# leggedrobotics/open3d_slam_private

Measured on AMD Instinct MI355X. Metric: ICP iterations/sec (scan-to-map), higher is better.
Workload: dtype f32

## Files before the change

### include/o3dslam_reg_debug.h

```cpp
#ifndef O3DSLAM_REG_DEBUG_H
#define O3DSLAM_REG_DEBUG_H

#include "o3dslam_reg.h"

#ifdef __cplusplus
extern "C" {
#endif

typedef struct {
    int32_t struct_size;
    int32_t profile_loop;
    int32_t match_variant;
    int32_t debug_flags;
    int32_t disable_halo;
    int32_t lanes_per_point;
    int32_t disable_fused;
    int32_t reserved;
} reg_debug_params;

REG_API reg_status reg_debug_configure(reg_handle* h, const reg_debug_params* d);

REG_API reg_status reg_debug_halo_bound(reg_handle* h, const float* xyz, int64_t n, float* out);

REG_API reg_status reg_debug_halo_witness(reg_handle* h, const float* xyz, int64_t n, int32_t* out);

REG_API reg_status reg_debug_live_resources(int64_t out[4]);

#ifdef __cplusplus
}
#endif
#endif
```

### open3d_slam_private_amd/capi.py

```python
from __future__ import annotations

import ctypes as C
import math
import os
import subprocess
import weakref

import numpy as np

_HERE = os.path.dirname(os.path.abspath(__file__))
_SO = os.environ.get("O3D_REG_LIB") or os.path.join(_HERE, "lib", "libo3dslam_reg.so")

STATUS_NAMES = {0: "OK", 1: "EMPTY_TARGET", 2: "EMPTY_SOURCE", 3: "NO_CORRESPONDENCES", 4: "BAD_TRANSFORM",
                5: "NOT_CONFIGURED", 6: "BAD_ARGUMENT", 7: "MISSING_FIELD", 8: "DEVICE_ERROR", 9: "UNSUPPORTED",
                10: "OUT_OF_BOUNDS"}
OUT_OF_BOUNDS = 10
COST_P2PL, COST_GICP = 0, 1
COST_O3D_P2PL, COST_O3D_P2P = 2, 3
SMOOTH_LEN_MAX = 15


class RegError(RuntimeError):
    def __init__(self, status, msg=""):
        self.status = status
# ... 276 lines not shown
def host_scan_key(seed: int, index: int) -> int:
    return int(load_library().reg_host_scan_key(int(seed), int(index)))


def default_scan_params(**overrides) -> ScanParams:
    p = ScanParams()
    load_library().reg_default_scan_params(C.byref(p))
    for k, v in overrides.items():
        if k in ("wide", "narrow"):
            v = Registration._crop_struct(v if v is not None else {"type": CROP_NONE})
        elif not hasattr(p, k):
            raise TypeError(f"unknown scan parameter {k}")
        setattr(p, k, v)
    p.struct_size = C.sizeof(ScanParams)
    return p


def host_ransac_est_k(est_k, confidence, count, k, ransac_n) -> float:
    return float(load_library().reg_host_ransac_est_k(float(est_k), float(confidence), int(count), int(k), int(ransac_n)))


class OctreeOut(C.Structure):
    _fields_ = [("xyz", C.c_void_p), ("normals", C.c_void_p), ("covs", C.c_void_p), ("src_idx", C.c_void_p),
                ("leaf_id", C.c_void_p), ("leaf_depth", C.c_void_p)]


class PmChain(C.Structure):
    _fields_ = [("struct_size", C.c_int32), ("knn", C.c_int32), ("minimizer", C.c_int32), ("use_robust", C.c_int32),
                ("robust_fct", C.c_int32), ("tuning", C.c_float), ("scale_estimator", C.c_int32),
                ("nb_iter_for_scale", C.c_int32), ("distance_type", C.c_int32), ("approximation", C.c_float),
                ("reserved", C.c_int32 * 2),
                ("use_min_dist_filter", C.c_int32), ("outlier_min_dist", C.c_float),
                ("use_median_dist", C.c_int32), ("median_factor", C.c_float),
                ("use_var_trimmed", C.c_int32), ("var_min_ratio", C.c_float), ("var_max_ratio", C.c_float),
                ("var_lambda", C.c_float)]


class PmChainV3(PmChain):
    _fields_ = [("with_cov", C.c_int32), ("sensor_std_dev", C.c_float),
                ("use_bound", C.c_int32), ("max_rotation_norm", C.c_float), ("max_translation_norm", C.c_float),
                ("bound_after_counter", C.c_int32),
                ("degeneracy_method", C.c_int32), ("sr_threshold", C.c_float), ("sr_use2019", C.c_int32),
                ("reserved2", C.c_int32)]


class MinimizerStats(C.Structure):
    _fields_ = [("struct_size", C.c_int32), ("returned_prior", C.c_int32), ("point_used_ratio", C.c_double),
                ("weighted_point_used_ratio", C.c_double), ("overlap", C.c_double), ("residual_error", C.c_double),
                ("n_rejected_matches", C.c_int64), ("n_rejected_points", C.c_int64)]


class TernaryXicp(C.Structure):
    _fields_ = [("struct_size", C.c_int32), ("enabled", C.c_int32), ("high_information", C.c_float),
                ("enough_information", C.c_float), ("insufficient_information", C.c_float),
                ("min_alignment_angle_deg", C.c_float), ("strong_alignment_angle_deg", C.c_float), ("reserved", C.c_int32)]


class TernaryXicpResult(C.Structure):
    _fields_ = [("struct_size", C.c_int32), ("iteration", C.c_int32), ("category", C.c_int32 * 6), ("sane", C.c_int32),
                ("reserved", C.c_int32), ("combined", C.c_double * 6), ("high", C.c_double * 6),
                ("n_combined", C.c_int64 * 6), ("n_high", C.c_int64 * 6), ("n_pairs", C.c_int64),
                ("constraint", C.c_float * 6), ("partial_sums", (C.c_double * 9) * 6), ("eigenvectors", (C.c_float * 9) * 2)]


TERNARY_LOCALIZABLE, TERNARY_PARTIAL_MIXED, TERNARY_PARTIAL_HIGH, TERNARY_NONE = 0, 1, 2, 3
PM_CHAIN_SIZE_V1 = 48
PM_CHAIN_SIZE_V2 = 80
DEGENERACY_NONE, DEGENERACY_SOLUTION_REMAPPING = 0, 1
PM_POINT_TO_PLANE, PM_POINT_TO_POINT = 0, 1
ROBUST_FCTS = {"cauchy": 0, "welsch": 1, "sc": 2, "gm": 3, "tukey": 4, "huber": 5, "L1": 6, "student": 7}
SCALE_ESTIMATORS = {"none": 0, "mad": 1, "berg": 2, "std": 3}
DISTANCE_TYPES = {"point2point": 0, "point2plane": 1}


EXPORTS = ["reg_default_params", "reg_shipped_params", "reg_create", "reg_destroy", "reg_last_error",
           "reg_set_stream", "reg_set_target", "reg_set_source", "reg_register", "reg_compute", "reg_prepare",
           "reg_linearize", "reg_get_correspondences", "reg_match_local", "reg_trim_histogram", "reg_reduce_local",
           "reg_solve_update", "reg_host_solve6", "reg_host_x_to_T", "reg_host_centroid", "reg_get_target_info", "reg_profile_kernels", "reg_source_centroid_sums", "reg_prepare_centroid", "reg_compose",
           "reg_dist_begin", "reg_dist_buffers", "reg_dist_phase", "reg_dist_finish",
           "reg_dist_fused_buffers", "reg_dist_poll", "reg_estimate_normals", "reg_smooth_normals", "reg_host_solve6_xicp",
           "reg_set_target_f64", "reg_get_target_source_indices", "reg_voxelize_within_volume", "reg_carve_indices", "reg_dist_xicp_buffers", "reg_dist_gather_buffers",
           "reg_dist_record", "reg_dist_centroid_sums", "reg_dist_prepare",
           "reg_information_matrix", "reg_set_source_f64", "reg_debug_configure", "reg_debug_halo_bound", "reg_debug_halo_witness",
           "reg_debug_live_resources",
           "reg_dist_get_unique_id", "reg_dist_init", "reg_dist_init_custom", "reg_dist_register", "reg_dist_shutdown",
           "reg_dist_info", "reg_dist_steer_create", "reg_dist_steer_destroy", "reg_dist_steer_step",
           "reg_dist_steer_counts", "reg_host_tail_plan", "reg_host_o3d_update",
           "reg_default_pm_chain", "reg_check_pm_chain", "reg_set_pm_chain", "reg_get_robust_state",
           "reg_get_correspondences_k", "reg_host_robust_weights", "reg_host_pm_p2p_update",
           "reg_get_var_trim", "reg_host_var_trim",
           "reg_get_covariance", "reg_get_covariance_sums", "reg_host_censi_covariance", "reg_get_minimizer_stats",
           "reg_get_degeneracy", "reg_get_bound", "reg_host_solution_remap",
           "reg_default_ternary_xicp", "reg_check_ternary_xicp", "reg_set_ternary_xicp", "reg_get_ternary_xicp",
           "reg_host_ternary_decide", "reg_host_partial_constraint", "reg_host_solve6_xicp_rhs",
           "reg_default_ssn_params", "reg_sampling_surface_normal", "reg_filter_points",
           "reg_default_octree_params", "reg_octree_grid", "reg_host_octree_root", "reg_host_octree_random_picks",
           "reg_filter_cloud", "reg_host_glibc_rand", "reg_default_voxel_grid_params", "reg_voxel_grid",
           "reg_overlap_indices", "reg_set_pair_overlap_f64", "reg_get_source_source_indices",
           "reg_compute_fpfh", "reg_match_features", "reg_ransac_correspondences", "reg_host_ransac_est_k",
           "reg_voxel_down_sample", "reg_random_down_sample", "reg_host_scan_key", "reg_default_scan_params",
           "reg_process_scan",
           "reg_dense_map_create", "reg_dense_map_destroy", "reg_dense_map_clear", "reg_dense_map_insert",
           "reg_default_dense_scan_params", "reg_dense_map_insert_scan", "reg_default_dense_carve_params",
           "reg_dense_map_carve", "reg_dense_map_transform", "reg_dense_map_center", "reg_dense_map_get_info",
           "reg_dense_map_export", "reg_dedup_voxels", "reg_host_dense_offsets"]


def lib_path() -> str:
    return _SO


def build_library(force: bool = False) -> str:
    src_dir = os.path.join(_HERE, "csrc")
    cmd = ["make", "-C", src_dir]
    if force:
        cmd.append("-B")
    subprocess.check_call(cmd)
    return _SO


_lib = None


def load_library():
    global _lib
    if _lib is not None:
        return _lib
    if not os.path.exists(_SO):
        raise ImportError(f"{_SO} is missing: build it with `python -c 'import __graft_entry__ as g; g.build()'` "
                          "(hipcc --offload-arch=gfx950).  There is no CPU fallback for the registration path.")
    lib = C.CDLL(_SO)
    vp, i64, f32p = C.c_void_p, C.c_int64, C.c_void_p
    lib.reg_create.argtypes = [C.POINTER(RegParams), C.POINTER(vp)]
    lib.reg_destroy.argtypes = [vp]
    lib.reg_last_error.argtypes = [vp]
    lib.reg_last_error.restype = C.c_char_p
    lib.reg_set_stream.argtypes = [vp, vp]
    lib.reg_debug_configure.argtypes = [vp, C.POINTER(RegDebugParams)]
    lib.reg_debug_halo_bound.argtypes = [vp, f32p, i64, f32p]
    lib.reg_debug_halo_witness.argtypes = [vp, f32p, i64, vp]
    lib.reg_debug_live_resources.argtypes = [C.POINTER(C.c_int64)]
    lib.reg_dist_get_unique_id.argtypes = [C.c_char_p]
    lib.reg_dist_init.argtypes = [vp, C.c_char_p, C.c_int, C.c_int]
    lib.reg_dist_init_custom.argtypes = [vp, C.POINTER(Collectives), C.c_int, C.c_int]
    lib.reg_dist_register.argtypes = [vp, f32p, f32p, C.POINTER(RegResult)]
    lib.reg_dist_shutdown.argtypes = [vp]
    lib.reg_dist_info.argtypes = [vp, C.POINTER(C.c_int64), C.POINTER(C.c_int32), C.POINTER(C.c_int32), C.POINTER(C.c_int32)]
    lib.reg_dist_steer_create.argtypes = [C.c_int, C.c_int, C.c_int, C.c_float, C.c_int]
    lib.reg_dist_steer_create.restype = vp
    lib.reg_dist_steer_destroy.argtypes = [vp]
    lib.reg_dist_steer_destroy.restype = None
    lib.reg_dist_steer_step.argtypes = [vp, C.POINTER(DistReply)]
    lib.reg_dist_steer_step.restype = DistAction
    lib.reg_dist_steer_counts.argtypes = [vp, C.POINTER(C.c_int32), C.POINTER(C.c_int32), C.POINTER(C.c_int32)]
    lib.reg_dist_steer_counts.restype = None
    lib.reg_set_source_f64.argtypes = [vp, vp, vp, vp, i64, C.c_int]
    lib.reg_set_target.argtypes = [vp, f32p, i64, f32p, i64, f32p, i64, C.c_int]
    lib.reg_set_source.argtypes = [vp, f32p, i64, f32p, i64, f32p, i64, C.c_int]
    lib.reg_register.argtypes = [vp, f32p, f32p, C.POINTER(RegResult)]
    lib.reg_compute.argtypes = [vp, f32p, i64, f32p, i64, f32p, i64, C.c_int, f32p, f32p, C.POINTER(RegResult)]
    lib.reg_prepare.argtypes = [vp, f32p]
    lib.reg_linearize.argtypes = [vp, f32p, f32p, f32p, C.POINTER(C.c_double), C.POINTER(C.c_int64)]
    lib.reg_get_correspondences.argtypes = [vp, vp, vp, vp]
    lib.reg_match_local.argtypes = [vp, f32p]
    lib.reg_trim_histogram.argtypes = [vp, C.c_int, C.c_uint32, vp]
    lib.reg_reduce_local.argtypes = [vp, f32p, C.c_float, vp]
    lib.reg_solve_update.argtypes = [C.POINTER(RegParams), vp, f32p, f32p, C.POINTER(C.c_int32)]
    lib.reg_host_solve6.argtypes = [f32p, f32p, f32p]
    lib.reg_host_solve6.restype = C.c_int
    lib.reg_host_x_to_T.argtypes = [f32p, f32p]
    lib.reg_host_solve6_xicp.argtypes = [f32p, f32p, vp, f32p]
    lib.reg_host_solve6_xicp.restype = C.c_int
    lib.reg_set_target_f64.argtypes = [vp, vp, vp, vp, i64, C.c_int, C.POINTER(RegCrop), C.POINTER(C.c_int64)]
    lib.reg_get_target_source_indices.argtypes = [vp, vp]
    lib.reg_carve_indices.argtypes = [vp, vp, vp, i64, vp, i64, C.c_int, C.POINTER(C.c_double), C.POINTER(RegCrop),
                                      C.c_double, C.c_double, C.c_double, C.c_double, vp, C.POINTER(C.c_int64)]
    lib.reg_voxelize_within_volume.argtypes = [vp, vp, vp, vp, i64, C.c_int, C.POINTER(RegCrop), C.c_double, vp, vp, vp,
                                               C.POINTER(C.c_int64), C.POINTER(C.c_int64)]
    lib.reg_overlap_indices.argtypes = [vp, vp, i64, vp, i64, C.c_int, C.POINTER(C.c_double), C.c_double, C.c_int32, vp,
                                        C.POINTER(C.c_int64), vp, C.POINTER(C.c_int64)]
    lib.reg_set_pair_overlap_f64.argtypes = [vp, vp, vp, vp, i64, vp, vp, vp, i64, C.c_int, C.POINTER(C.c_double), C.c_double,
                                             C.c_int32, C.POINTER(C.c_int64), C.POINTER(C.c_int64)]
    lib.reg_get_source_source_indices.argtypes = [vp, vp]
    lib.reg_compute_fpfh.argtypes = [vp, vp, i64, vp, i64, i64, C.c_int, C.c_int, C.c_float, vp, vp, vp, C.POINTER(C.c_int64)]
    lib.reg_match_features.argtypes = [vp, vp, i64, vp, i64, C.c_int, C.c_int, vp, vp, vp, C.POINTER(C.c_int64)]
    lib.reg_ransac_correspondences.argtypes = [vp, vp, i64, vp, i64, vp, i64, C.c_int, C.POINTER(RansacParams),
                                               C.POINTER(RansacResult), vp, vp]
    lib.reg_host_ransac_est_k.argtypes = [C.c_double, C.c_double, i64, i64, C.c_int32]
    lib.reg_host_ransac_est_k.restype = C.c_double
    lib.reg_voxel_down_sample.argtypes = [vp, vp, vp, vp, i64, C.c_int, C.c_double, vp, vp, vp, C.POINTER(C.c_int64)]
    lib.reg_random_down_sample.argtypes = [vp, vp, vp, vp, i64, C.c_int, C.c_double, C.c_uint64, vp, vp, vp, vp,
                                           C.POINTER(C.c_int64)]
    lib.reg_host_scan_key.argtypes = [C.c_uint64, C.c_uint64]
    lib.reg_host_scan_key.restype = C.c_uint64
    lib.reg_default_scan_params.argtypes = [C.POINTER(ScanParams)]
    lib.reg_default_scan_params.restype = None
    lib.reg_process_scan.argtypes = [vp, vp, vp, vp, i64, C.c_int, C.POINTER(ScanParams), vp, vp, vp, C.POINTER(ScanResult)]
    pd16, pi64 = C.POINTER(C.c_double), C.POINTER(C.c_int64)
    lib.reg_dense_map_create.argtypes = [vp, C.c_double, C.POINTER(vp)]
    lib.reg_dense_map_destroy.argtypes = [vp]
    lib.reg_dense_map_destroy.restype = None
    lib.reg_dense_map_clear.argtypes = [vp]
    lib.reg_dense_map_insert.argtypes = [vp, vp, vp, vp, i64, C.c_int, pd16, pi64, pi64]
    lib.reg_default_dense_scan_params.argtypes = [C.POINTER(DenseScanParams)]
    lib.reg_default_dense_scan_params.restype = None
    lib.reg_dense_map_insert_scan.argtypes = [vp, vp, vp, vp, i64, C.c_int, C.POINTER(DenseScanParams), pd16, pi64, pi64]
    lib.reg_default_dense_carve_params.argtypes = [C.POINTER(DenseCarveParams)]
    lib.reg_default_dense_carve_params.restype = None
    lib.reg_dense_map_carve.argtypes = [vp, vp, i64, C.c_int, pd16, C.POINTER(DenseCarveParams), vp, pi64]
    lib.reg_dense_map_transform.argtypes = [vp, pd16]
    lib.reg_dense_map_center.argtypes = [vp, pd16]
    lib.reg_dense_map_get_info.argtypes = [vp, C.POINTER(DenseMapInfo)]
    lib.reg_dense_map_export.argtypes = [vp, C.c_int, vp, vp, vp, vp, vp, i64, pi64]
    lib.reg_dedup_voxels.argtypes = [vp, vp, i64, C.c_int, C.c_double, vp, pi64]
    lib.reg_host_dense_offsets.argtypes = [C.c_double, C.c_double, vp]
    lib.reg_host_dense_offsets.restype = C.c_int32
    lib.reg_host_centroid.argtypes = [f32p, i64, i64, f32p]
    lib.reg_host_o3d_update.argtypes = [C.c_int, vp, vp, C.POINTER(C.c_int32)]
    lib.reg_get_target_info.argtypes = [vp, C.POINTER(TargetInfo)]
    lib.reg_profile_kernels.argtypes = [vp, f32p, C.c_int, f32p]
    lib.reg_source_centroid_sums.argtypes = [vp, vp]
    lib.reg_prepare_centroid.argtypes = [vp, f32p, f32p]
    lib.reg_compose.argtypes = [vp, f32p, f32p]
    lib.reg_dist_begin.argtypes = [vp, f32p]
# ... 872 lines not shown
            out["normals"] = np.zeros((n, 3), np.float32)
        if cv is not None:
            out["covs"] = np.zeros((n, 6), np.float32)
        o = OctreeOut()
        for key in ("xyz", "normals", "covs", "src_idx", "leaf_id", "leaf_depth"):
            setattr(o, key, out[key].ctypes.data if key in out else None)
        m = C.c_int64(0)
        self._check(self._lib.reg_octree_grid(self._h, _ptr(xyz), xyz.shape[1] if xyz.ndim == 2 else 3, _ptr(nr), _ptr(cv),
                                              n, 0, C.byref(p), C.byref(o), C.byref(m)))
        for key in ("xyz", "src_idx", "normals", "covs"):
            if key in out:
                out[key] = out[key][:m.value].copy()
        out["n_out"] = int(m.value)
        return out

    def octree_grid_device(self, xyz_ptr, xyz_stride, n, params: "OctreeParams", xyz_out_ptr, nrm_ptr=None, cov_ptr=None,
                           normals_out_ptr=None, covs_out_ptr=None, src_idx_ptr=None, leaf_id_ptr=None,
                           leaf_depth_ptr=None) -> int:
        o = OctreeOut(xyz_out_ptr, normals_out_ptr, covs_out_ptr, src_idx_ptr, leaf_id_ptr, leaf_depth_ptr)
        m = C.c_int64(0)
        self._check(self._lib.reg_octree_grid(self._h, C.c_void_p(xyz_ptr), xyz_stride, nrm_ptr, cov_ptr, n, 1,
                                              C.byref(params), C.byref(o), C.byref(m)))
        return int(m.value)

    def smooth_normals(self, normals, ids):
        nr = np.ascontiguousarray(normals, dtype=np.float32).copy()
        ii = np.ascontiguousarray(ids, dtype=np.int32)
        passes = C.c_int32(0)
        self._check(self._lib.reg_smooth_normals(self._h, _ptr(nr), _ptr(ii), nr.shape[0], ii.shape[1], 0, C.byref(passes)))
        return nr, int(passes.value)

    def estimate_normals_device(self, xyz_ptr, xyz_stride, n, normals_ptr, k=10, max_dist=np.inf, viewpoint=None,
                                regularise=False, eigvals_ptr=None, covs_ptr=None, ids_ptr=None, eigvecs_ptr=None,
                                densities_ptr=None, mean_dists_ptr=None):
        vp_ = _f32(viewpoint) if viewpoint is not None else None
        o = NormalsOut()
        o.normals, o.eigvals, o.eigvecs, o.covs = normals_ptr, eigvals_ptr, eigvecs_ptr, covs_ptr
        o.densities, o.mean_dists, o.ids = densities_ptr, mean_dists_ptr, ids_ptr
        resc = C.c_int64(0)
        self._check(self._lib.reg_estimate_normals(
            self._h, C.c_void_p(xyz_ptr), xyz_stride, n, 1, int(k), float(max_dist), _ptr(vp_), 1 if regularise else 0,
            C.byref(o), C.byref(resc)))
        return int(resc.value)

    def set_target_device(self, xyz_ptr, xyz_stride, m, nrm_ptr=None, nrm_stride=3, cov_ptr=None):
        self._check(self._lib.reg_set_target(self._h, C.c_void_p(xyz_ptr), xyz_stride,
                                             C.c_void_p(nrm_ptr) if nrm_ptr else None, nrm_stride,
                                             C.c_void_p(cov_ptr) if cov_ptr else None, m, 1))

    def set_source_device(self, xyz_ptr, xyz_stride, n, nrm_ptr=None, nrm_stride=3, cov_ptr=None):
        self._check(self._lib.reg_set_source(self._h, C.c_void_p(xyz_ptr), xyz_stride,
                                             C.c_void_p(nrm_ptr) if nrm_ptr else None, nrm_stride,
                                             C.c_void_p(cov_ptr) if cov_ptr else None, n, 1))
        self.n_source = n

    def register(self, T_init=None):
        Ti = _T_in(np.eye(4) if T_init is None else T_init)
        To = np.zeros(16, np.float32)
        res = RegResult()
        st = self._lib.reg_register(self._h, _ptr(Ti), _ptr(To), C.byref(res))
        self.last_result = res
        self._check(st)
        return _T_out(To), res

    def information_matrix(self, T, max_dist):
        Ti = _T_in(T)
        info = (C.c_double * 36)()
        n = C.c_int64(0)
        self._check(self._lib.reg_information_matrix(self._h, _ptr(Ti), float(max_dist), info, C.byref(n)))
        return np.array(info[:], np.float64).reshape(6, 6), int(n.value)

    def halo_bound(self, xyz):
        x = _f32(xyz)
        out = np.empty(x.shape[0], np.float32)
        self._check(self._lib.reg_debug_halo_bound(self._h, _ptr(x), x.shape[0], _ptr(out)))
        return out

    def halo_witness(self, xyz):
        x = _f32(xyz)
        out = np.empty(x.shape[0], np.int32)
        self._check(self._lib.reg_debug_halo_witness(self._h, _ptr(x), x.shape[0], _ptr(out)))
        return out

    def prepare(self, T_init=None):
        Ti = _T_in(np.eye(4) if T_init is None else T_init)
        self._check(self._lib.reg_prepare(self._h, _ptr(Ti)))

    def linearize(self, T_iter=None):
        Ti = _T_in(np.eye(4) if T_iter is None else T_iter)
        H = np.zeros(36, np.float32)
        b = np.zeros(6, np.float32)
        err = C.c_double()
        cnt = C.c_int64()
        self._check(self._lib.reg_linearize(self._h, _ptr(Ti), _ptr(H), _ptr(b), C.byref(err), C.byref(cnt)))
        return H.reshape(6, 6), b, err.value, cnt.value

    def correspondences(self, want_w=True):
        n = self.n_source
        ids = np.empty(n, np.int32)
        d2 = np.empty(n, np.float32)
        w = np.empty(n, np.float32) if want_w else None
        self._check(self._lib.reg_get_correspondences(self._h, _ptr(ids), _ptr(d2), _ptr(w)))
        return ids, d2, w

    def set_pm_chain(self, chain: "PmChain | None"):
        if chain is not None:
            chain.struct_size = C.sizeof(type(chain))
        self.pm_chain = chain
        self._check(self._lib.reg_set_pm_chain(self._h, C.byref(chain) if chain is not None else None))

    def set_ternary_xicp(self, ternary: "TernaryXicp | None"):
        if ternary is not None:
            ternary.struct_size = C.sizeof(TernaryXicp)
        self._check(self._lib.reg_set_ternary_xicp(self._h, C.byref(ternary) if ternary is not None else None))
        self.ternary_xicp = ternary

    def get_ternary_xicp(self) -> TernaryXicpResult:
        out = TernaryXicpResult()
        out.struct_size = C.sizeof(TernaryXicpResult)
        self._check(self._lib.reg_get_ternary_xicp(self._h, C.byref(out)))
        return out

    def get_correspondences_k(self, knn=None, want_w=True):
        if knn is None:
            knn = self.pm_chain.knn if getattr(self, "pm_chain", None) is not None else 1
        n = self.n_source
        ids = np.empty((n, knn), np.int32)
        d2 = np.empty((n, knn), np.float32)
        w = np.empty((n, knn), np.float32) if want_w else None
        self._check(self._lib.reg_get_correspondences_k(self._h, int(knn), _ptr(ids), _ptr(d2), _ptr(w)))
        return ids, d2, w

    def robust_state(self):
        sc = C.c_float()
        it = C.c_int32()
        self._check(self._lib.reg_get_robust_state(self._h, C.byref(sc), C.byref(it)))
        return float(sc.value), int(it.value)

    def get_var_trim(self):
        ratio, k, n = C.c_float(), C.c_int64(), C.c_int64()
        self._check(self._lib.reg_get_var_trim(self._h, C.byref(ratio), C.byref(k), C.byref(n)))
        return float(ratio.value), int(k.value), int(n.value)

    def get_covariance(self):
        cov = np.zeros(36, np.float32)
        rank = C.c_int32()
        self._check(self._lib.reg_get_covariance(self._h, _ptr(cov), C.byref(rank)))
        return cov.reshape(6, 6), int(rank.value)

    def get_covariance_sums(self):
        Hp, Mp = np.zeros(21, np.float64), np.zeros(21, np.float64)
        self._check(self._lib.reg_get_covariance_sums(self._h, _ptr(Hp), _ptr(Mp)))
        return unpack_sym6(Hp), unpack_sym6(Mp)

    def get_minimizer_stats(self) -> MinimizerStats:
        st = MinimizerStats()
        st.struct_size = C.sizeof(MinimizerStats)
        self._check(self._lib.reg_get_minimizer_stats(self._h, C.byref(st)))
        return st

    def get_degeneracy(self):
        cat, eig, cond = np.zeros(6, np.int32), np.zeros(6, np.float32), C.c_float()
        self._check(self._lib.reg_get_degeneracy(self._h, _ptr(cat), _ptr(eig), C.byref(cond)))
        return cat, eig, float(cond.value)

    def get_bound(self):
# ... 253 lines not shown
        return self._lib.reg_dist_steer_step(self._s, C.byref(reply) if reply is not None else None)

    def counts(self):
        g, f, s = C.c_int32(), C.c_int32(), C.c_int32()
        self._lib.reg_dist_steer_counts(self._s, C.byref(g), C.byref(f), C.byref(s))
        return g.value, f.value, s.value

    def __del__(self):
        try:
            if self._s:
                self._lib.reg_dist_steer_destroy(self._s)
                self._s = None
        except Exception:
            pass


def solve_update(params: RegParams, sums, T_iter):
    lib = load_library()
    s = np.ascontiguousarray(sums, np.float64)
    To = np.zeros(16, np.float32)
    rank = C.c_int32()
    st = lib.reg_solve_update(C.byref(params), _ptr(s), _ptr(_T_in(T_iter)), _ptr(To), C.byref(rank))
    if st != 0:
        raise RegError(st, "reg_solve_update")
    return _T_out(To), rank.value


def host_solve6(A, b):
    x = np.zeros(6, np.float32)
    rank = load_library().reg_host_solve6(_ptr(_f32(A).reshape(36)), _ptr(_f32(b)), _ptr(x))
    return x, rank


def host_solve6_xicp(A, b, flags):
    x = np.zeros(6, np.float32)
    f = np.ascontiguousarray(flags, np.int32)
    rank = load_library().reg_host_solve6_xicp(_ptr(_f32(A).reshape(36)), _ptr(_f32(b)), _ptr(f), _ptr(x))
    return x, rank


def host_x_to_T(x):
    T = np.zeros(16, np.float32)
    load_library().reg_host_x_to_T(_ptr(_f32(x)), _ptr(T))
    return _T_out(T)


def host_centroid(xyz):
    xyz = _f32(xyz)
    out = np.zeros(3, np.float32)
    load_library().reg_host_centroid(_ptr(xyz), xyz.shape[1], xyz.shape[0], _ptr(out))
    return out


def host_o3d_update(cost, sums):
    s = np.ascontiguousarray(sums, np.float64).reshape(32)
    U = np.zeros(16, np.float64)
    rank = C.c_int32()
    st = load_library().reg_host_o3d_update(int(cost), _ptr(s), _ptr(U), C.byref(rank))
    if st != 0:
        raise RegError(st, "reg_host_o3d_update")
    return U.reshape(4, 4).T.copy(), rank.value


def host_tail_plan(n, cus=256, tile=0):
    lib = load_library()
    lib.reg_host_tail_plan.argtypes = [C.c_int64, C.c_int32, C.c_int32, C.POINTER(C.c_int32)]
    lib.reg_host_tail_plan.restype = None
    out = (C.c_int32 * 4)()
    lib.reg_host_tail_plan(int(n), int(cus), int(tile), out)
    return bool(out[0]), int(out[1]), int(out[2]), int(out[3])


def host_predict_band(limit, prev=math.inf, prev2=math.inf, last_count=0, last_lo=math.inf, last_hi=math.inf, debug_narrow=0):
    lib = load_library()
    lib.reg_host_predict_band.argtypes = [C.c_float, C.c_float, C.c_float, C.c_uint32, C.c_float, C.c_float, C.c_int32,
                                          C.POINTER(C.c_float), C.POINTER(C.c_float)]
    lib.reg_host_predict_band.restype = None
    out = (C.c_float * 2)()
    lib.reg_host_predict_band(float(limit), float(prev), float(prev2), int(last_count), float(last_lo), float(last_hi),
                              int(debug_narrow), out, None)
    return np.float32(out[0]), np.float32(out[1])


def host_band_constants():
    lib = load_library()
    lib.reg_host_predict_band.argtypes = [C.c_float, C.c_float, C.c_float, C.c_uint32, C.c_float, C.c_float, C.c_int32,
                                          C.POINTER(C.c_float), C.POINTER(C.c_float)]
    lib.reg_host_predict_band.restype = None
    c = (C.c_float * 8)()
    lib.reg_host_predict_band(math.inf, math.inf, math.inf, 0, math.inf, math.inf, 0, None, c)
    names = ("band_cap", "wide_rel", "floor", "ratio_max", "centre_gain", "geom_rel", "guard_frac", "forced_wide")
    return {k: float(np.float32(v)) for k, v in zip(names, c)}
```

### open3d_slam_private_amd/csrc/host_handle.hpp

```cpp
#pragma once

struct EnvSwitches {
    bool trace = false;
    bool event_timing = false;
    bool halo_occ = true;
    bool no_dynprune = false;
    bool no_empty_bound = false;
    bool no_witness = false;
    bool no_burst = false;
    bool hints = false;
    bool stamps = false;
    bool coh_stats = false;
    bool tail_always = false;
    bool update_generic = false;
    bool no_tail = false;
    int tail_wpc = 0;
    double dist_timeout_s = 30.0;
    float tail_timeout_s = 2.f;
    int xcd_tile_first = 32;
    int xcd_tile_later = 16;
    float settle_trans = 0.02f;
    float settle_rot = 4e-3f;
    int tail_min_iters = 8;
    int tail_tile = 0;
    bool no_gicp_tail = false;
    int gicp_tail_after = 1;
    float tail_settle_tol = 1.2f;
    int lookahead = 2;
    float settle_tol = 0.05f;
    float halo_ratio = 1.25f;
    float halo_rho = 0.4f;
    float reach_bins = 7.25f;
    float bin_occupancy = 8.f;
    float level_ratio = 2.0f;
    void read() {
        trace = getenv("O3D_TRACE") != nullptr;
        event_timing = getenv("O3D_EVENT_TIMING") != nullptr;
        no_burst = getenv("O3D_NO_BURST") != nullptr;
        no_dynprune = getenv("O3D_NO_DYNPRUNE") != nullptr;
        no_empty_bound = getenv("O3D_NO_EMPTY_BOUND") != nullptr;
        no_witness = getenv("O3D_NO_WITNESS") != nullptr;
        halo_occ = getenv("O3D_NO_HALO_OCC") == nullptr;
        hints = getenv("O3D_HINTS") != nullptr;
        stamps = getenv("O3D_STAMPS") != nullptr;
        coh_stats = getenv("O3D_COH_STATS") != nullptr;
        tail_always = getenv("O3D_TAIL_ALWAYS") != nullptr;
        no_tail = getenv("O3D_NO_TAIL") != nullptr;
        if (const char* v = getenv("O3D_UPDATE_GENERIC")) update_generic = atoi(v) != 0;
        if (const char* v = getenv("O3D_TAIL_WPC")) tail_wpc = std::max(0, atoi(v));
        if (const char* v = getenv("O3D_DIST_TIMEOUT_S")) dist_timeout_s = std::max(0.5, atof(v));
        if (const char* v = getenv("O3D_TAIL_SETTLE")) tail_settle_tol = (float)atof(v);
        if (const char* v = getenv("O3D_NO_GICP_TAIL")) no_gicp_tail = atoi(v) != 0;
        if (const char* v = getenv("O3D_TAIL_TILE")) tail_tile = std::max(0, atoi(v));
        if (const char* v = getenv("O3D_TAIL_MIN_ITERS")) tail_min_iters = std::max(0, atoi(v));
        if (const char* v = getenv("O3D_SETTLE_TRANS")) settle_trans = (float)atof(v);
        if (const char* v = getenv("O3D_SETTLE_ROT")) settle_rot = (float)atof(v);
        if (const char* v = getenv("O3D_XCD_TILE_FIRST")) xcd_tile_first = std::max(0, atoi(v));
        if (const char* v = getenv("O3D_XCD_TILE_LATER")) xcd_tile_later = std::max(0, atoi(v));
        if (const char* v = getenv("O3D_GICP_TAIL_AFTER")) gicp_tail_after = atoi(v);
        if (const char* v = getenv("O3D_TAIL_TIMEOUT_S")) tail_timeout_s = std::min(30.f, std::max(0.01f, (float)atof(v)));
        if (const char* v = getenv("O3D_KAHEAD")) lookahead = std::max(1, atoi(v));
        if (const char* v = getenv("O3D_SETTLE")) settle_tol = (float)atof(v);
        if (const char* v = getenv("O3D_HALO_RATIO")) halo_ratio = std::min(4.0f, std::max(0.5f, (float)atof(v)));
        if (const char* v = getenv("O3D_HALO_RHO")) halo_rho = std::min(1.0f, std::max(0.05f, (float)atof(v)));
        if (const char* v = getenv("O3D_REACH_BINS")) reach_bins = std::max(1.0f, (float)atof(v));
        if (const char* v = getenv("O3D_BIN_OCC")) bin_occupancy = std::min(64.0f, std::max(1.0f, (float)atof(v)));
        if (const char* v = getenv("O3D_LEVEL_RATIO")) level_ratio = std::min(4.0f, std::max(1.2f, (float)atof(v)));
    }
};

struct DistCtx;

struct reg_handle {
    reg_params prm;
    reg_debug_params dbg;
    EnvSwitches env;
    std::string err;
    Stream stream;
    Event ev0, ev1, ev_iter, ev_s0, ev_s1;
    Event ev_p0, ev_p1;
    std::vector<Event> prof_ev;
    Pinned<HostMirror> h_mirror;
    Pinned<IterState> h_iter;
    Pinned<PrepState> h_prep;
    bool device_ok = false;
    bool structure_only = false;
    reg_handle* normals_ws = nullptr;
    DevBuf n_out, n_ids, n_extra, n_mom;
    DevBuf fp_xyz, fp_nrm, fp_ids, fp_cnt, fp_out, fp_misc, mf_a, mf_b, mf_part, mf_nn, mf_flags;
    DevBuf rs_src, rs_tgt, rs_cor, rs_pairs, rs_batch, rs_part, rs_rec;
    std::vector<RsRecord> rs_head;
    DevBuf i_xicp;
    DevBuf c_in_xyz, c_in_nrm, c_in_cov, c_flags, c_offs, c_xyz, c_nrm, c_cov, c_idx;
    DevBuf r_in_xyz, r_in_nrm, r_in_cov, r_xyz, r_nrm, r_cov;
    int64_t crop_kept = 0;
    DevBuf v_fout, v_oout, v_out;
    DevBuf v_ukeys, v_ustart;
    DevBuf ov_keys[2], ov_sorted, ov_ukeys[2], ov_ucnt[2], ov_flags[2], ov_offs[2], ov_misc, ov_sidx;
    DevBuf i_info;
    int64_t src_kept = 0;
    DevBuf sp_in[3], sp_a[3], sp_b[3], sp_c[3], sp_f32[3], sp_keys, sp_keys2, sp_vals, sp_vals2, sp_flags, sp_offs, sp_part,
        sp_misc;
    DevBuf dm_in[3], dm_crop[3], dm_tf[2], dm_keys, dm_keys2, dm_vals, dm_vals2, dm_heads, dm_run, dm_rank, dm_new, dm_newoff,
        dm_newkeys, dm_mark, dm_keep, dm_off1, dm_off2, dm_misc, dm_out;
    DevBuf d_d2all;
    int64_t dist_nmax = 0;
    int dist_gather_ranks = 0;
    bool xicp_pending = false;
    bool src_prep_pending = false;
    float source_prep_ms = 0.f;
    int rotation_corrected = 0;
    bool iter_copy_pending = false;

    int64_t m = 0;
    bool has_tnrm = false, has_tcov = false;
    float c_ref[3] = {0, 0, 0};
    float t_mid[3] = {0, 0, 0};
    DevBuf t_raw, t_nrm_raw, t_cov_raw, t_centred, t_keys, t_keys2, t_vals, t_vals2, t_pts, t_nrm, t_cov, t_flags,
        t_scan, t_hash, t_cells, t_misc, t_dir, t_rows;
    DevBuf rp_tmp;
    Grid grid;
    reg_target_info info;
    float target_build_ms = 0.f;

    int64_t n = 0;
    bool has_snrm = false, has_scov = false, prepared = false;
    int64_t s_stride = 3, s_nstride = 3;
    float c_read[3] = {0, 0, 0};
    DevBuf s_raw, s_nrm_raw, s_cov_raw, s_xyz, s_nrm, s_cov, s_misc;
    float T_init[16];
    float T0[16];
    DevBuf i_pos, i_d2, i_w, i_hist, i_state, i_partials, i_sums, i_ids;
    DevBuf i_iter;
    unsigned long long seq = 0;
    DevBuf t_halo_start, t_halo_cursor, t_halo_pts, t_halo_dir, i_band, i_acc, i_cache, i_stats, i_queue, i_qcount;
    DevBuf s_prep;
    int cent_slot = 0;
    bool prep_pending = false;
    DevBuf i_hint, s_keys, s_keys2, s_perm, s_perm2, s_tmp, i_tmpf;
    const uint32_t* perm = nullptr;
    int last_stalls = 0;
    int64_t n_total_hint = 0;
    int match_launches = 0;
    int tail_sync_slot = 0, tail_sync_last = 0;
    bool tail_sync_dirty = true;
    int last_tail_launches = 0, last_tail_iters = 0;
    DevBuf i_tail_sync, i_tail_rows, i_tail_band;
    unsigned long long dist_seq0 = 0;
    DevBuf d_contrib, d_gathered;
    int dist_ranks = 0, dist_rank = 0;
    DistCtx* dist = nullptr;
    unsigned long long src_epoch = 0;
    std::vector<int> prof_kind;
    bool profiling = false;
    int shift0 = 21;
    int n_blocks = 0;
    bool have_match = false;
    bool pm_on = false;
    reg_pm_chain pm;
    bool pm_have_match = false;
    DevBuf pm_pos, pm_d2, pm_w, pm_keys, pm_hist, pm_sel, pm_state, pm_partials;
    DevBuf pm_sorted, pm_sort_tmp, pm_var;
    size_t pm_sort_bytes = 0;
    DevBuf pm_xstate, pm_xrows, pm_xmeans, pm_xcov;
    PmExtraState pm_xhost;
    PmCovOut pm_cov_host;
    bool pm_x_valid = false;
    bool pm_cov_valid = false;
    float pm_cov_ms = 0.f;
    double pm_last_error = 0.0;
    bool xt_on = false;
    reg_ternary_xicp xt;
    DevBuf xt_state, xt_rows;
    XtState xt_host;
    bool xt_valid = false;
    DevBuf f_in, f_in_nrm, f_in_cov, f_px, f_pn, f_pc, f_perm, f_keys, f_keys2, f_segs, f_boxes, f_boxes2, f_leaf,
        f_mom, f_mom2, f_lid, f_keep, f_pos, f_misc, f_out;
    DevBuf f_fields, f_draws;
    DevBuf o_keys, o_keys_s, o_iota, o_idx, o_idx2, o_rank, o_rank_a, o_rank_s, o_c, o_kk, o_heads, o_pos, o_open, o_depth,
        o_start, o_rand, o_radii;
};
static_assert(!std::is_copy_constructible<DevBuf>::value && !std::is_copy_constructible<reg_handle>::value, "owners are not copied");

#define HIPCHK(h, call)                                                                        \
    do {                                                                                       \
        hipError_t e_ = (call);                                                                \
        if (e_ != hipSuccess) {                                                                \
            (h)->err = std::string(#call) + ": " + hipGetErrorString(e_);                      \
            return REG_DEVICE_ERROR;                                                           \
        }                                                                                      \
    } while (0)

static inline void col_to_row(const float* c, float* r) { m4_transpose(c, r); }
static inline void row_to_col(const float* r, float* c) { m4_transpose(r, c); }

static inline int grid_for(int64_t n, int block = 256) { return (int)((n + block - 1) / block); }

static inline bool cost_is_o3d(int cost) { return cost == REG_COST_O3D_P2PL || cost == REG_COST_O3D_P2P; }

static inline bool pm_needs_tnrm(const reg_handle* h) {
    return h->pm.minimizer == REG_PM_POINT_TO_PLANE || h->prm.use_surface_normal ||
           (h->pm.use_robust && h->pm.distance_type == REG_DIST_POINT2PLANE);
}

static reg_status check_target_fields(reg_handle* h, bool has_nrm, bool has_cov) {
    if ((h->prm.cost == REG_COST_P2PL || h->prm.cost == REG_COST_O3D_P2PL) && !has_nrm && !h->structure_only &&
        !(h->pm_on && !pm_needs_tnrm(h))) {
        h->err = "InvalidField: point-to-plane needs the `normals` descriptor on the reference";
        return REG_MISSING_FIELD;
    }
    if (h->prm.cost == REG_COST_GICP && !has_cov && !h->structure_only) {
        h->err = "InvalidField: GICP needs covariances on the reference";
        return REG_MISSING_FIELD;
    }
    return REG_OK;
}
static reg_status check_source_fields(reg_handle* h, bool has_nrm, bool has_cov) {
    if (h->prm.cost == REG_COST_P2PL && h->prm.use_surface_normal && !has_nrm) {
        h->err = "InvalidField: SurfaceNormalOutlierFilter needs the `normals` descriptor on the reading";
        return REG_MISSING_FIELD;
    }
    if (h->prm.cost == REG_COST_GICP && !has_cov) {
        h->err = "InvalidField: GICP needs covariances on the reading";
        return REG_MISSING_FIELD;
    }
    return REG_OK;
}

extern "C" {
// ... 203 lines not shown
```

### open3d_slam_private_amd/csrc/host_loop.hpp

```cpp
#pragma once


static reg_status check_ready(reg_handle* h, bool need_prepared) {
    if (!h) return REG_BAD_ARGUMENT;
    if (!h->device_ok) return REG_DEVICE_ERROR;
    if (h->m == 0) {
        h->err = "no reference set (reg_set_target)";
        return REG_NOT_CONFIGURED;
    }
    if (h->n == 0) {
        h->err = "no reading set (reg_set_source)";
        return REG_NOT_CONFIGURED;
    }
    if (need_prepared && !h->prepared) {
        h->err = "reg_prepare has not been called for this reading";
        return REG_NOT_CONFIGURED;
    }
    return REG_OK;
}

static reg_status prepare_rowmajor(reg_handle* h, const float* T_init_row, const float* c_override = nullptr,
                                   int64_t n_global = 0, const IterState* init_state = nullptr) {
    reg_status s = check_ready(h, false);
    if (s != REG_OK) return s;
// ... 63 lines not shown
}


static void xicp_frame_change(const reg_handle* h, float Trd12[12]) {
    float A[16], Trd[16];
    m4_identity(A);
    for (int k = 0; k < 3; ++k) A[4 * k + 3] = -h->c_ref[k];
    m4_mul(A, h->T_init, Trd);
    for (int k = 0; k < 12; ++k) Trd12[k] = Trd[k];
}

static reg_status build_iter_state(reg_handle* h, const float* T_row, int update, IterState* st) {
    std::memset(st, 0, sizeof(IterState));
    for (int i = 0; i < 16; ++i) {
        st->T[i] = T_row[i];
        st->Td[i] = (double)T_row[i];
    }
    st->chk = Checkers();
    st->chk.max_iter = h->prm.max_iter;
    st->chk.min_diff_rot = h->prm.min_diff_rot;
    st->chk.min_diff_trans = h->prm.min_diff_trans;
    st->chk.smooth_len = h->prm.smooth_len;
    st->chk.init(T_row);
    st->cost = h->prm.cost;
    st->fixed_iters = h->prm.fixed_iters;
    st->max_iter = h->prm.max_iter;
    st->update = update;
    st->gicp_rot_eps = h->prm.gicp_rot_eps;
    st->gicp_trans_eps = h->prm.gicp_trans_eps;
    st->gicp_stop_rule = h->prm.gicp_stop_rule;
    st->gicp_rel_fitness = h->prm.gicp_rel_fitness;
    st->gicp_rel_rmse = h->prm.gicp_rel_rmse;
    st->n_total = (float)(h->n_total_hint > 0 ? h->n_total_hint : h->n);
    st->band_lo = st->band_hi = INFINITY;
    st->limit_last = st->limit_prev = st->limit_prev2 = INFINITY;
    st->use_trim = (h->prm.cost == REG_COST_P2PL && h->prm.use_trimmed) ? 1 : 0;
    st->trim_ratio = h->prm.trim_ratio;
    st->band_cap = kBandCap;
    st->qcount = h->i_qcount.as<unsigned int>();
    st->debug_narrow_band = ((h->dbg.debug_flags & 8) ? 1 : 0) | ((h->dbg.debug_flags & 64) ? 2 : 0);
    h->xicp_pending = false;
    for (int k = 0; k < 6; ++k) st->xicp_flags[k] = 1;
    if (h->prm.use_xicp && h->prm.cost == REG_COST_P2PL && update) {
        HIPCHK(h, h->i_xicp.reserve(sizeof(XicpState)));
        st->xicp_stage = 1;
        st->xicp_enough = h->prm.xicp_enough;
        st->xicp_insufficient = h->prm.xicp_insufficient;
        st->xicp_cos_min = (float)std::cos((double)h->prm.xicp_min_angle_deg * 3.14159265358979323846 / 180.0);
        st->xicp_cos_strong = (float)std::cos((double)h->prm.xicp_strong_angle_deg * 3.14159265358979323846 / 180.0);
        xicp_frame_change(h, st->xicp_Trd);
        h->xicp_pending = true;
    }
    return REG_OK;
}

static reg_status init_iter_state(reg_handle* h, const float* T_row, int update) {
    IterState* st = h->h_iter;
    if (h->iter_copy_pending) HIPCHK(h, hipEventSynchronize(h->ev_iter));
    reg_status s = build_iter_state(h, T_row, update, st);
    if (s != REG_OK) return s;
    HIPCHK(h, hipMemcpyAsync(h->i_iter.p, st, sizeof(IterState), hipMemcpyHostToDevice, h->stream));
    HIPCHK(h, hipEventRecord(h->ev_iter, h->stream));
    h->iter_copy_pending = true;
    return REG_OK;
}

static reg_status enqueue_match(reg_handle* h, bool zero_hist = false) {
    const bool trim = h->prm.cost == REG_COST_P2PL && h->prm.use_trimmed;
    if (trim && zero_hist) HIPCHK(h, hipMemsetAsync(h->i_hist.p, 0, 3 * 2048 * 4, h->stream));
    const bool fused_hist = h->dbg.match_variant == 3;
    uint32_t* hist0 = (trim && fused_hist) ? h->i_hist.as<uint32_t>() : nullptr;
    uint32_t* hist2 = trim ? h->i_hist.as<uint32_t>() + 4096 : nullptr;
    const IterState* it = h->i_iter.as<IterState>();
    if (h->dbg.match_variant == 1) {
        prof_mark(h, 0, true);
        k_match<<<h->n_blocks, 256, 0, h->stream>>>(h->s_xyz.as<float4>(), h->n, it, h->grid, h->i_pos.as<int>(),
                                                    h->i_d2.as<float>(), hist0, hist2, h->shift0);
        prof_mark(h, 0, false);
    } else {
        uint8_t* hint = h->dbg.match_variant == 2 ? nullptr : h->i_hint.as<uint8_t>();
        const int lanes = h->dbg.lanes_per_point == 4 ? 4 : (h->dbg.lanes_per_point == 2 ? 2 : 8);
        const int blocks = grid_for(h->n * lanes);
        const int tile = h->match_launches < 2 ? h->env.xcd_tile_first : h->env.xcd_tile_later;
        ++h->match_launches;
        const dim3 grid(xcd_tiled_grid(blocks, tile)), block(256);
        auto go = [&](auto kernel) {
            launch_timed(h, 0, kernel, grid, block, 0, (const float4*)h->s_xyz.as<float4>(), h->n, it, h->grid,
                         h->i_pos.as<int>(), h->i_d2.as<float>(), hist0, hist2, hint, h->shift0, h->dbg.debug_flags, blocks,
                         h->i_cache.as<float4>(), tile);
        };
        if (lanes == 4)
            go(k_match_g8<4>);
        else if (lanes == 2)
            go(k_match_g8<2>);
        else
            go(k_match_g8<8>);
    }
    h->have_match = true;
    return REG_OK;
}

static void enqueue_select(reg_handle* h) {
    const float* d2 = h->i_d2.as<float>();
    uint32_t* hist = h->i_hist.as<uint32_t>();
    SelectState* st = h->i_state.as<SelectState>();
    const int hb = std::min(h->n_blocks, 128);
    if (h->dbg.match_variant != 3) launch_hist_level0(h, d2, h->n, hb, hist);
    launch_select_level(h, 1, d2, h->n, hb, hist, st, h->prm.trim_ratio);
    launch_select_level(h, 2, d2, h->n, hb, hist, st, h->prm.trim_ratio);
}

static reg_status enqueue_linearize(reg_handle* h, bool want_w, bool limit_from_state = false) {
    float* w = want_w ? h->i_w.as<float>() : nullptr;
    if (h->prm.cost == REG_COST_P2PL) {
        launch_linearize_p2pl(h, h->prm.use_trimmed ? (limit_from_state ? 1 : 2) : 0, w);
    } else if (cost_is_o3d(h->prm.cost)) {
        const IterState* it = h->i_iter.as<IterState>();
        const float3 o = make_float3(h->t_mid[0], h->t_mid[1], h->t_mid[2]);
        if (h->prm.cost == REG_COST_O3D_P2PL)
            k_linearize_o3d<REG_COST_O3D_P2PL><<<h->n_blocks, 256, 0, h->stream>>>(
                h->s_xyz.as<float4>(), h->n, it, h->i_pos.as<int>(), h->i_d2.as<float>(), h->t_nrm.as<float4>(), o, w,
                h->i_partials.as<double>());
        else
            k_linearize_o3d<REG_COST_O3D_P2P><<<h->n_blocks, 256, 0, h->stream>>>(
                h->s_xyz.as<float4>(), h->n, it, h->i_pos.as<int>(), h->i_d2.as<float>(), h->t_pts.as<float4>(), o, w,
                h->i_partials.as<double>());
        update_o3d_from_partials(h);
        return REG_OK;
    } else {
        launch_linearize_gicp(h, w);
    }
    update_from_partials(h);
    if (h->xicp_pending) {
        h->xicp_pending = false;
        launch_xicp_center(h, h->i_pos.as<int>(), h->i_w.as<float>());
        launch_xicp_detect(h, h->i_pos.as<int>(), h->i_w.as<float>());
        update_xicp_finish(h);
    }
    return REG_OK;
}

static reg_status enqueue_fused(reg_handle* h) {
    CohStats* stats = h->env.coh_stats ? h->i_stats.as<CohStats>() : nullptr;
    const int rows = h->dbg.lanes_per_point == 4 ? launch_fused_search<4>(h, h->i_band.as<float>(), (int)kBandCap, stats, true)
                                                 : launch_fused_search<8>(h, h->i_band.as<float>(), (int)kBandCap, stats, true);
    update_fused_from_band(h, rows);
    h->have_match = true;
    return REG_OK;
}

constexpr int kTailMaxDevices = 64;
static std::mutex g_tail_mutex[kTailMaxDevices];
static std::atomic<int> g_reg_active[kTailMaxDevices];
struct RegActiveGuard {
    int dev;
    explicit RegActiveGuard(int d) : dev(d >= 0 && d < kTailMaxDevices ? d : -1) {
        if (dev >= 0) g_reg_active[dev].fetch_add(1, std::memory_order_relaxed);
    }
    ~RegActiveGuard() {
        if (dev >= 0) g_reg_active[dev].fetch_sub(1, std::memory_order_relaxed);
    }
    bool alone() const { return dev >= 0 && g_reg_active[dev].load(std::memory_order_relaxed) == 1; }
};
static int g_tail_cus[kTailMaxDevices];
static std::mutex g_tail_probe_mutex;

struct TailPlan {
    bool ok = false;
    int grid = 0, wpc = 0, chunk8 = 0, tile = 0;
};

static int tail_device_cus(int dev) {
    if (dev < 0 || dev >= kTailMaxDevices) return -1;
    std::lock_guard<std::mutex> lk(g_tail_probe_mutex);
    if (g_tail_cus[dev] != 0) return g_tail_cus[dev];
    int cus = 0, nb = 0;
    hipError_t e = hipDeviceGetAttribute(&cus, hipDeviceAttributeMultiprocessorCount, dev);
    int nb2 = 0;
    if (e == hipSuccess)
        e = hipFuncSetAttribute(reinterpret_cast<const void*>(k_tail<false>), hipFuncAttributeMaxDynamicSharedMemorySize, kTailLdsBytes);
    if (e == hipSuccess)
        e = hipFuncSetAttribute(reinterpret_cast<const void*>(k_tail<true>), hipFuncAttributeMaxDynamicSharedMemorySize, kTailLdsBytes);
    if (e == hipSuccess)
        e = hipOccupancyMaxActiveBlocksPerMultiprocessor(&nb, reinterpret_cast<const void*>(k_tail<false>), kTailThreads, kTailLdsBytes);
    if (e == hipSuccess)
        e = hipOccupancyMaxActiveBlocksPerMultiprocessor(&nb2, reinterpret_cast<const void*>(k_tail<true>), kTailThreads, kTailLdsBytes);
    g_tail_cus[dev] = (e == hipSuccess && nb >= kTailWgsPerCu && nb2 >= kTailWgsPerCu && cus >= 8) ? cus : -1;
    (void)hipGetLastError();
    return g_tail_cus[dev];
}

static TailPlan tail_plan_for(int64_t n, int cus, int wpc_cap, int tile) {
    TailPlan pl;
    if (cus < 8 || n <= 0) return pl;
    int wpc_max = cus * kTailWgsPerCu / 8;
    if (wpc_cap > 0) wpc_max = std::min(wpc_max, wpc_cap);
    pl.wpc = (int)std::max<int64_t>(1, std::min<int64_t>(wpc_max, (n + 2047) / 2048));
    pl.tile = std::max(0, tile);
    const int64_t unit = 8 * (int64_t)std::max(1, pl.tile);
    pl.chunk8 = (int)((((n + 7) / 8) + unit - 1) / unit * unit);
    const int64_t octets = pl.chunk8 / 8, per_wg = (octets + pl.wpc - 1) / pl.wpc * 8;
    pl.grid = 8 * pl.wpc;
    pl.ok = per_wg <= kTailSlots;
    return pl;
}
static TailPlan tail_plan(const reg_handle* h) {
    if (cost_is_o3d(h->prm.cost)) return TailPlan();
    if (h->prm.cost == REG_COST_GICP && h->env.no_gicp_tail) return TailPlan();
    if (h->dbg.disable_fused == 1 || (h->dbg.debug_flags & (16 | 64 | 128)) || h->dbg.lanes_per_point == 4 || h->env.no_tail)
        return TailPlan();
    return tail_plan_for(h->n, tail_device_cus(h->prm.device), h->env.tail_wpc, h->env.tail_tile);
}

static void last_step_motion(const HostMirror* m, float* trans, float* rot) {
    const float* A = m->T;
    const float* B = m->T_prev;
    float R[9];
    for (int i = 0; i < 3; ++i)
        for (int j = 0; j < 3; ++j) R[3 * i + j] = A[4 * i + 0] * B[4 * j + 0] + A[4 * i + 1] * B[4 * j + 1] + A[4 * i + 2] * B[4 * j + 2];
    float t[3];
    for (int i = 0; i < 3; ++i) t[i] = A[4 * i + 3] - (R[3 * i + 0] * B[3] + R[3 * i + 1] * B[7] + R[3 * i + 2] * B[11]);
    *trans = std::sqrt(t[0] * t[0] + t[1] * t[1] + t[2] * t[2]);
    const float sx = 0.5f * (R[7] - R[5]), sy = 0.5f * (R[2] - R[6]), sz = 0.5f * (R[3] - R[1]);
    *rot = std::sqrt(sx * sx + sy * sy + sz * sz);
}

static reg_status enqueue_tail(reg_handle* h, const TailPlan& pl, int max_iters) {
    if (!h->i_tail_sync.p) h->tail_sync_dirty = true;
    HIPCHK(h, h->i_tail_sync.reserve(2 * (size_t)kTailSyncBytes));
    if (h->tail_sync_dirty) {
        HIPCHK(h, hipMemsetAsync(h->i_tail_sync.p, 0, 2 * (size_t)kTailSyncBytes, h->stream));
        h->tail_sync_dirty = false;
    }
    const int sync_slot = h->tail_sync_slot;
    h->tail_sync_slot ^= 1;
    h->tail_sync_last = sync_slot;
    unsigned* const sync_cur = h->i_tail_sync.as<unsigned>() + (size_t)sync_slot * (kTailSyncBytes / 4);
    unsigned* const sync_next = h->i_tail_sync.as<unsigned>() + (size_t)(sync_slot ^ 1) * (kTailSyncBytes / 4);
    HIPCHK(h, h->i_tail_rows.reserve((size_t)2 * pl.grid * kTailHistRow * 8));
    HIPCHK(h, h->i_tail_band.reserve((size_t)2 * kTailBandCap * kTailRec * 4));
    const FilterCfg f = make_filter_cfg(h, 0);
    TailCfg cfg;
    cfg.n = h->n;
    cfg.chunk8 = pl.chunk8;
    cfg.wpc = pl.wpc;
    cfg.tile = pl.tile;
    cfg.max_iters = std::max(1, std::min(max_iters, kTailMaxIters));
    cfg.slack = coherent_slack(h);
    cfg.seq = ++h->seq;
    cfg.timeout_ticks = (unsigned long long)(h->env.tail_timeout_s * 1e8);
    uint8_t* hint = h->dbg.match_variant == 2 ? nullptr : h->i_hint.as<uint8_t>();
    const bool gicp = h->prm.cost == REG_COST_GICP;
    const float4* s_attr = gicp ? (const float4*)h->s_cov.as<float4>() : (const float4*)(h->has_snrm ? h->s_nrm.as<float4>() : nullptr);
    const float4* t_attr = gicp ? (const float4*)h->t_cov.as<float4>() : (const float4*)h->t_nrm.as<float4>();
    auto go = [&](auto kernel) {
        launch_timed(h, 3, kernel, dim3(pl.grid), dim3(kTailThreads), kTailLdsBytes, (const float4*)h->s_xyz.as<float4>(), s_attr,
                     h->i_iter.as<IterState>(), h->grid, t_attr, f, h->i_pos.as<int>(), h->i_d2.as<float>(), h->i_w.as<float>(), hint,
                     h->i_cache.as<float4>(), sync_cur, h->i_tail_rows.as<double>(), h->i_tail_band.as<float>(), h->h_mirror.dev, cfg,
                     sync_next);
    };
    if (gicp)
        go(k_tail<true>);
    else
        go(k_tail<false>);
    HIPCHK(h, hipGetLastError());
    h->have_match = true;
    return REG_OK;
}

static reg_status enqueue_iteration(reg_handle* h, bool want_w) {
    reg_status s = enqueue_match(h);
    if (s != REG_OK) return s;
    if (h->prm.cost == REG_COST_P2PL && h->prm.use_trimmed) enqueue_select(h);
    return enqueue_linearize(h, want_w);
}

static inline unsigned long long mirror_seq(const reg_handle* h) {
    return __atomic_load_n(&h->h_mirror->seq, __ATOMIC_ACQUIRE);
}

static reg_status wait_seq(reg_handle* h, unsigned long long seq) {
    for (unsigned spins = 0;; ++spins) {
        if (mirror_seq(h) >= seq) return REG_OK;
        __builtin_ia32_pause();
        if ((spins & 0x3fff) == 0x3fff) {
            hipError_t e = hipStreamQuery(h->stream);
            if (e == hipSuccess) return REG_OK;
            if (e != hipErrorNotReady) {
                h->err = std::string("device fault while waiting for the iteration: ") + hipGetErrorString(e);
                return REG_DEVICE_ERROR;
            }
        }
    }
}

static reg_status iterate_once(reg_handle* h, const float* T_row, bool want_w) {
    reg_status s = init_iter_state(h, T_row, 0);
    if (s != REG_OK) return s;
    s = enqueue_iteration(h, want_w);
    if (s != REG_OK) return s;
    s = wait_seq(h, h->seq);
    if (s != REG_OK) return s;
    HIPCHK(h, hipGetLastError());
    return REG_OK;
}

static void sums_to_system(const double* sums, int cost, float* H, float* b) {
    if (cost == REG_COST_O3D_P2P) {
        std::memset(H, 0, 36 * sizeof(float));
        std::memset(b, 0, 6 * sizeof(float));
        return;
    }
    const bool p2pl = cost == REG_COST_P2PL;
    int k = 0;
    for (int a = 0; a < 6; ++a)
        for (int c = a; c < 6; ++c) {
            const float v = (float)sums[k++];
            H[6 * a + c] = v;
            H[6 * c + a] = v;
        }
    for (int a = 0; a < 6; ++a) b[a] = p2pl ? -(float)sums[21 + a] : (float)sums[21 + a];
}

static void compose_rowmajor(reg_handle* h, const float* T_iter, float* Tout_row, bool later_kernel_reported = false) {
    if (h->prep_pending) {
        if (!later_kernel_reported) (void)hipStreamSynchronize(h->stream);
        std::memcpy(h->c_read, h->h_prep->c_read, 12);
        std::memcpy(h->T0, h->h_prep->T0, 64);
        h->prep_pending = false;
    }
    if (h->prm.cost == REG_COST_P2PL) {
// ... 68 lines not shown
    }
    void acknowledge() {
        acked = std::max(acked, m_seq);
        completed = any ? h->h_mirror->iterations : 0;
        inflight = (int)(h->seq - acked);
    }
    reg_status wait_next() {
        const reg_status s = wait_seq(h, acked + 1);
        if (s != REG_OK) return s;
        if (mirror_seq(h) <= acked) {
            if (hipStreamQuery(h->stream) == hipSuccess && mirror_seq(h) <= acked) acked = h->seq;
        }
        return REG_OK;
    }
};

struct SteerInput {
    bool any;
    float limit_last, limit_prev, step_trans, step_rot;
    int completed, inflight, generic_left, limit;
};
struct SteerPolicy {
    bool trimming, can_fuse, p2pl, no_burst;
    bool use_tail = false, tail_off = false;
    int tail_min_iters, fixed;
    float fused_settle_tol, tail_settle_tol, settle_trans, settle_rot;
    explicit SteerPolicy(const reg_handle* h) {
        p2pl = h->prm.cost == REG_COST_P2PL;
        can_fuse = p2pl && h->dbg.disable_fused != 1;
        trimming = p2pl && h->prm.use_trimmed && h->prm.trim_ratio != 1.0f;
        no_burst = h->env.no_burst;
        fixed = h->prm.fixed_iters;
        tail_min_iters = fixed > 0 ? 0 : h->env.tail_min_iters;
        fused_settle_tol = h->env.settle_tol;
        tail_settle_tol = h->env.tail_settle_tol;
        settle_trans = h->env.settle_trans;
        settle_rot = h->env.settle_rot;
    }
};
struct SteerChoice {
    enum Kind { kGeneric, kFused, kTail } kind;
    int count;
};

static SteerChoice steer_choose(const SteerInput& in, const SteerPolicy& p) {
    const bool tail_now = p.use_tail && !p.tail_off && in.completed + in.inflight >= p.tail_min_iters;
    const float settle_tol = tail_now ? p.tail_settle_tol : p.fused_settle_tol;
    bool settled = true;
    if (p.trimming) {
        settled = in.any && in.limit_prev < INFINITY && in.limit_last < INFINITY &&
                  std::fabs(in.limit_last - in.limit_prev) <= settle_tol * in.limit_last;
    }
    if (settled && in.any && (p.p2pl || p.fixed <= 0) && (p.can_fuse || tail_now)) {
        if (in.step_trans > p.settle_trans || in.step_rot > p.settle_rot) settled = false;
    }
    if (!(p.can_fuse || tail_now) || in.generic_left > 0 || !settled) return {SteerChoice::kGeneric, 1};
    const int rest = in.limit - (in.completed + in.inflight);
    if (tail_now) return {SteerChoice::kTail, rest};
    return {SteerChoice::kFused, p.fixed > 0 && !p.no_burst ? rest : 1};
}

static reg_status wait_tail(reg_handle* h, unsigned long long tail_seq, Lookahead& la, bool* tail_off) {
    const HostMirror* mir = h->h_mirror;
    for (unsigned spins = 0;; ++spins) {
        const unsigned long long m = mirror_seq(h);
        if (m >= tail_seq) break;
        if (m + 1 == tail_seq) {
            const HostMirror::SeqRecord* rec = &mir->ring[(tail_seq - 1) % kSeqRing];
            if (__atomic_load_n(&rec->seq, __ATOMIC_ACQUIRE) == tail_seq - 1 && (rec->done || rec->stall)) break;
        }
        __builtin_ia32_pause();
        if ((spins & 0xfff) == 0xfff) {
            const hipError_t e = hipStreamQuery(h->stream);
            if (e == hipSuccess) break;
            if (e != hipErrorNotReady) {
                h->tail_sync_dirty = true;
                h->err = std::string("device fault while waiting for the tail kernel: ") + hipGetErrorString(e);
                return REG_DEVICE_ERROR;
            }
        }
    }
    const bool reported = mirror_seq(h) >= tail_seq;
    const unsigned* sync_last = h->i_tail_sync.as<unsigned>() + (size_t)h->tail_sync_last * (kTailSyncBytes / 4);
    unsigned words[4] = {0, 0, 0, 0};
    if (!reported || h->env.coh_stats || mir->status == REG_DEVICE_ERROR)
        (void)hipMemcpy(words, sync_last + kTailErrWord, sizeof(words), hipMemcpyDeviceToHost);
    if (words[0] != 0 || (reported && mir->status == REG_DEVICE_ERROR)) {
        h->tail_sync_dirty = true;
        h->err = "persistent tail kernel: a grid barrier timed out (workgroups not co-resident? another process "
                 "running a persistent kernel on this GPU?); set O3D_NO_TAIL=1 to use the three-launch iteration";
        return REG_DEVICE_ERROR;
    }
    if (!reported && !(mir->stall && std::max(mirror_seq(h), la.seq0) > la.acked)) la.acked = h->seq;
    if (h->env.coh_stats)
        fprintf(stderr, "[o3dreg] tail launch: %u iterations, %u point searches (%.2f %% of the point-iterations), stall cause %u, band records of its last iteration %d\n", words[2],
                words[1], words[2] ? 100.0 * words[1] / ((double)words[2] * (double)h->n) : 0.0, words[3], reported ? mir->pad_nband : -1);
    if (reported) h->last_tail_iters += mir->pad3;
    if (reported && mir->stall && h->prm.fixed_iters <= 0) *tail_off = true;
#if O3D_TAIL_STAMPS
    {
        unsigned long long st[24];
        (void)hipMemcpy(st, sync_last + kTailStampWord, sizeof(st), hipMemcpyDeviceToHost);
        const double it_n = std::max(1, reported ? mir->pad3 : 1);
        static const char* names[12] = {"check", "search", "epilogue", "bandrec+comps", "sum+publish+drain", "arrive+wait", "row sums",
                                        "band-stage", "band-scan", "band-rank", "band-add", "solve+update"};
        for (int wg = 0; wg < 2; ++wg) {
            fprintf(stderr, "[o3dreg] tail stamps (us per iteration, %s workgroup):", wg ? "last" : "first");
            for (int i = 0; i < 12; ++i) fprintf(stderr, " %s %.2f", names[i], st[12 * wg + i] * 0.01 / it_n);
            fprintf(stderr, "\n");
        }
    }
#endif
    return REG_OK;
}

static reg_status loop_time_end(reg_handle* h, bool event_timing, std::chrono::steady_clock::time_point t_begin, float* loop_ms) {
    if (event_timing) {
        HIPCHK(h, hipEventRecord(h->ev1, h->stream));
        HIPCHK(h, hipEventSynchronize(h->ev1));
        (void)hipEventElapsedTime(loop_ms, h->ev0, h->ev1);
    } else {
        *loop_ms = std::chrono::duration<float, std::milli>(std::chrono::steady_clock::now() - t_begin).count();
    }
    return REG_OK;
}

static void loop_end_diagnostics(reg_handle* h, reg_result* res) {
    const HostMirror* mir = h->h_mirror;
    if (h->env.hints) {
        std::vector<uint8_t> hv((size_t)h->n);
        if (hipMemcpy(hv.data(), h->i_hint.p, (size_t)h->n, hipMemcpyDeviceToHost) == hipSuccess) {
            long long cnt[18] = {0};
            for (uint8_t v : hv) ++cnt[v < 17 ? v : 17];
            fprintf(stderr, "[o3dreg] terminating level of the last iteration (halo, then levels with rho =");
            for (int l = 0; l < h->grid.n_levels; ++l) fprintf(stderr, " %.3f", h->grid.rho[l]);
            fprintf(stderr, "):");
            for (int l = 0; l <= h->grid.n_levels; ++l) fprintf(stderr, " %lld", cnt[l]);
            fprintf(stderr, "\n");
        }
    }
    if (h->env.coh_stats) {
        CohStats cs;
        if (hipMemcpy(&cs, h->i_stats.p, sizeof(cs), hipMemcpyDeviceToHost) == hipSuccess) {
            fprintf(stderr, "[o3dreg] coherent fused iterations: %llu point-iterations, %llu searched (%.2f %%)\n", cs.n_points,
                    cs.n_searched, cs.n_points ? 100.0 * (double)cs.n_searched / (double)cs.n_points : 0.0);
            (void)hipMemset(h->i_stats.p, 0, sizeof(cs));
        }
    }
    if (h->env.stamps) {
        fprintf(stderr, "update kernel stamps (cycles): reduce %llu [rows %llu select %llu band-add %llu] solve %llu update+check %llu mirror %llu\n", mir->stamps[0],
                mir->stamps[4], mir->stamps[5], mir->stamps[6], mir->stamps[1], mir->stamps[2], mir->stamps[3]);
        fprintf(stderr, "   select detail: verify+stage-issue %llu, zero+hist+barriers %llu, wave0 pick/rank %llu\n", mir->stamps[3], mir->stamps[7] >> 32, mir->stamps[7] & 0xffffffffull);
    }
    if (h->profiling) {
        for (size_t i = 0; i + 1 < h->prof_ev.size(); i += 2) {
            float ms = 0;
            if (hipEventElapsedTime(&ms, h->prof_ev[i], h->prof_ev[i + 1]) == hipSuccess) {
                const int kind = h->prof_kind[i / 2];
                res->prof_ms[kind] += ms;
                res->prof_launches[kind] += 1;
            }
        }
        h->prof_ev.clear();
        h->prof_kind.clear();
        h->profiling = false;
    }
}

static reg_status register_pm(reg_handle* h, const float* Ti, float T_out[16], reg_result* res);

extern "C" {

void reg_host_tail_plan(int64_t n, int32_t cus, int32_t tile, int32_t plan[4]) {
    const TailPlan pl = tail_plan_for(n, cus, 0, tile);
    plan[0] = pl.ok ? 1 : 0;
    plan[1] = pl.grid;
    plan[2] = pl.wpc;
    plan[3] = pl.chunk8;
}

REG_API void reg_host_predict_band(float limit, float prev, float prev2, uint32_t last_count, float last_lo, float last_hi,
                                   int32_t debug_narrow, float band[2], float consts[8]) {
    const Band b = predict_band(limit, prev, prev2, last_count, last_lo, last_hi, debug_narrow);
    if (band) {
        band[0] = b.lo;
        band[1] = b.hi;
    }
    if (consts) {
        const float c[8] = {(float)kTailBandCap, kTailWideRel, kBandFloor, kBandRatioMax, kBandCentreGain, kBandGeomRel, kBandGuardFrac,
                            kBandForcedWide};
        for (int i = 0; i < 8; ++i) consts[i] = c[i];
    }
}

reg_status reg_prepare(reg_handle* h, const float T_init[16]) {
    if (!h || !T_init) return REG_BAD_ARGUMENT;
    float Tr[16];
    col_to_row(T_init, Tr);
    return prepare_rowmajor(h, Tr);
}

reg_status reg_linearize(reg_handle* h, const float T_iter[16], float H[36], float b[6], double* err,
                         int64_t* n_inliers) {
    reg_status s = check_ready(h, true);
    if (s != REG_OK) return s;
    if (!T_iter) return REG_BAD_ARGUMENT;
    if (h->prm.cost == REG_COST_O3D_P2P) {
        h->err = "reg_linearize: point-to-point (Umeyama) has no normal equations";
        return REG_UNSUPPORTED;
    }
    if (h->pm_on) {
        h->err = "reg_linearize: not available with a libpointmatcher chain (reg_set_pm_chain)";
        return REG_UNSUPPORTED;
    }
    float Tr[16];
    col_to_row(T_iter, Tr);
    if (!m4_is_finite(Tr)) return REG_BAD_TRANSFORM;
    HIPCHK(h, hipSetDevice(h->prm.device));
    s = iterate_once(h, Tr, true);
    if (s != REG_OK) return s;
    const double* sums = h->h_mirror->sums;
    if (H && b) sums_to_system(sums, h->prm.cost, H, b);
    if (err) *err = sums[27];
    if (n_inliers) *n_inliers = (int64_t)llround(sums[28]);
    if (sums[28] == 0.0) {
        h->err = "ErrorMinimizer: no point to minimize";
        return REG_NO_CORRESPONDENCES;
    }
    return REG_OK;
}

reg_status reg_register(reg_handle* h, const float T_init[16], float T_out[16], reg_result* res) {
    if (!h || !T_init || !T_out) return REG_BAD_ARGUMENT;
    reg_result local;
    if (!res) res = &local;
    std::memset(res, 0, sizeof(*res));
    std::memcpy(T_out, T_init, 64);
    float Ti[16];
    col_to_row(T_init, Ti);
    const auto t_reg0 = std::chrono::steady_clock::now();
    auto rmark = [&](const char* what) {
        if (h->env.trace)
            fprintf(stderr, "[o3dreg] register %-14s t=%.1fus\n", what,
                    std::chrono::duration<double, std::micro>(std::chrono::steady_clock::now() - t_reg0).count());
    };
    if (h->pm_on) return register_pm(h, Ti, T_out, res);
    const bool p2pl = h->prm.cost == REG_COST_P2PL;
    float T_start[16];
    if (p2pl)
        m4_identity(T_start);
    else
        std::memcpy(T_start, Ti, 64);
    std::memcpy(h->T_init, Ti, 64);
    IterState st0;
    reg_status s = build_iter_state(h, T_start, 1, &st0);
    if (s != REG_OK) return s;
    rmark("iter state");
    s = prepare_rowmajor(h, Ti, nullptr, 0, &st0);
    if (s != REG_OK) return s;
    rmark("prepared");
    h->profiling = h->dbg.profile_loop != 0;
    h->prof_ev.clear(), h->prof_kind.clear();
    const bool event_timing = h->profiling || h->env.event_timing;
    if (event_timing) HIPCHK(h, hipEventRecord(h->ev0, h->stream));
    const auto t_loop_begin = std::chrono::steady_clock::now();
    rmark("ev0");
    Lookahead la{h, h->seq, h->seq};
    SteerPolicy pol(h);
    const TailPlan tail_pl = (pol.can_fuse || h->prm.cost == REG_COST_GICP) ? tail_plan(h) : TailPlan();
    const RegActiveGuard active(h->prm.device);
    std::unique_lock<std::mutex> tail_lock;
    if (tail_pl.ok && (active.alone() || h->env.tail_always)) {
        tail_lock = std::unique_lock<std::mutex>(g_tail_mutex[h->prm.device], std::try_to_lock);
    }
    pol.use_tail = tail_pl.ok && tail_lock.owns_lock();
    const int limit = sequence_limit(h->prm);
    const int kAhead = h->env.lookahead;
    const HostMirror* mir = h->h_mirror;
    int generic_left = pol.trimming ? 2 : (h->prm.cost == REG_COST_GICP ? std::max(1, h->env.gicp_tail_after) : 1);
    unsigned long long last_traced = 0;
    const auto t_loop0 = std::chrono::steady_clock::now();
    unsigned long long tail_seq = 0;
    h->last_stalls = h->last_tail_launches = h->last_tail_iters = 0;
    for (;;) {
        if (tail_seq) {
            s = wait_tail(h, tail_seq, la, &pol.tail_off);
            if (s != REG_OK) return s;
            tail_seq = 0;
            continue;
        }
        la.look();
        if (la.any && mir->done) break;
        if (la.any && mir->stall && la.m_seq > la.acked) {
            HIPCHK(h, hipStreamSynchronize(h->stream));
            la.acked = h->seq;
            generic_left = 2;
            ++h->last_stalls;
            continue;
        }
        if (h->env.trace && la.m_seq != last_traced) {
            last_traced = la.m_seq;
            float mt = 0.f, mr = 0.f;
            last_step_motion(mir, &mt, &mr);
            fprintf(stderr, "[o3dreg] seq %llu iter %d stall %d band_n %d limit %.6g prev %.6g band [%.6g, %.6g) step %.2e m %.2e rad\n",
                    la.m_seq - la.seq0, mir->iterations, mir->stall, mir->stall ? mir->band_count : mir->pad_nband, mir->limit_last,
                    mir->limit_prev, mir->band_lo, mir->band_hi, mt, mr);
        }
        la.acknowledge();
        if (la.completed + la.inflight < limit && la.inflight < kAhead) {
            SteerInput seen = {la.any, mir->limit_last, mir->limit_prev, 0.f, 0.f, la.completed, la.inflight, generic_left, limit};
            if (la.any) last_step_motion(mir, &seen.step_trans, &seen.step_rot);
            const SteerChoice c = steer_choose(seen, pol);
            const auto tq0 = std::chrono::steady_clock::now();
            if (c.kind == SteerChoice::kGeneric) {
                s = enqueue_iteration(h, true);
                if (generic_left > 0) --generic_left;
            } else if (c.kind == SteerChoice::kTail) {
                s = enqueue_tail(h, tail_pl, c.count);
                tail_seq = h->seq;
                ++h->last_tail_launches;
            } else {
                for (int burst = c.count; burst > 0 && s == REG_OK; --burst) s = enqueue_fused(h);
            }
            if (h->env.trace) {
                const auto tq1 = std::chrono::steady_clock::now();
                fprintf(stderr, "[o3dreg] t=%.1fus enqueue seq %llu (%s) took %.1fus; mirror at %llu\n",
                        std::chrono::duration<double, std::micro>(tq0 - t_loop0).count(), h->seq - la.seq0,
                        c.kind == SteerChoice::kGeneric ? "generic" : (c.kind == SteerChoice::kTail ? "tail" : "fused"),
                        std::chrono::duration<double, std::micro>(tq1 - tq0).count(), std::max(mirror_seq(h), la.seq0) - la.seq0);
            }
            if (s != REG_OK) return s;
            continue;
        }
        if (la.inflight == 0) break;
        s = la.wait_next();
        if (s != REG_OK) return s;
    }
    rmark("loop done");
    s = loop_time_end(h, event_timing, t_loop_begin, &res->loop_ms);
    if (s != REG_OK) return s;
    HIPCHK(h, hipGetLastError());
    rmark("loop timed");
    loop_end_diagnostics(h, res);
    s = write_result(h, h->prm.use_xicp != 0, true, (double)h->n, true, T_out, res);
    if (s != REG_OK) {
        h->err = mir->sums[29] == 0.0 ? "No matches available for computing distance quantiles"
                                      : "ErrorMinimizer: no point to minimize";
        return s;
    }
    res->n_band_stalls = h->last_stalls;
    res->n_tail_launches = h->last_tail_launches;
    res->n_tail_iterations = h->last_tail_iters;
    rmark("return");
    return REG_OK;
}

reg_status reg_information_matrix(reg_handle* h, const float T[16], float max_dist, double info[36], int64_t* n_pairs) {
    if (!h || !T || !info) return REG_BAD_ARGUMENT;
    if (n_pairs) *n_pairs = 0;
    if (!(max_dist > 0.f) || max_dist > h->prm.max_dist) {
        h->err = "reg_information_matrix: max_dist must be positive and within the handle's max_dist";
        return REG_BAD_ARGUMENT;
    }
    float Tr[16];
    col_to_row(T, Tr);
    reg_status s = prepare_rowmajor(h, Tr);
    if (s != REG_OK) return s;
    float T_start[16];
    if (h->prm.cost == REG_COST_P2PL)
        m4_identity(T_start);
    else
        std::memcpy(T_start, Tr, 64);
    s = init_iter_state(h, T_start, 0);
    if (s != REG_OK) return s;
    s = enqueue_match(h, false);
    if (s != REG_OK) return s;
    h->have_match = true;
    const int blocks = (int)std::min<int64_t>(512, (h->n + 255) / 256);
    HIPCHK(h, h->i_info.reserve((size_t)512 * 10 * sizeof(double)));
    HIPCHK(h, hipMemsetAsync(h->i_info.p, 0, (size_t)blocks * 10 * sizeof(double), h->stream));
    k_info_sums<<<blocks, 256, 0, h->stream>>>(h->i_pos.as<int>(), h->i_d2.as<float>(), h->n, h->t_pts.as<float4>(),
                                               h->c_ref[0], h->c_ref[1], h->c_ref[2], max_dist * max_dist,
                                               h->i_info.as<double>());
    std::vector<double> rows((size_t)blocks * 10);
    HIPCHK(h, hipMemcpyAsync(rows.data(), h->i_info.p, rows.size() * sizeof(double), hipMemcpyDeviceToHost, h->stream));
    HIPCHK(h, hipStreamSynchronize(h->stream));
    HIPCHK(h, hipGetLastError());
    double m[10] = {0, 0, 0, 0, 0, 0, 0, 0, 0, 0};
    for (int b = 0; b < blocks; ++b)
        for (int k = 0; k < 10; ++k) m[k] += rows[(size_t)b * 10 + k];
    const double c = m[0], sx = m[1], sy = m[2], sz = m[3], xx = m[4], yy = m[5], zz = m[6], xy = m[7], xz = m[8], yz = m[9];
    const double I[36] = {yy + zz, -xy, -xz, 0, -sz, sy,
                          -xy, xx + zz, -yz, sz, 0, -sx,
                          -xz, -yz, xx + yy, -sy, sx, 0,
                          0, sz, -sy, c, 0, 0,
                          -sz, 0, sx, 0, c, 0,
                          sy, -sx, 0, 0, 0, c};
// ... 50 lines not shown
```

### open3d_slam_private_amd/csrc/kernels_fused.hpp

```cpp
#pragma once

constexpr int kBandCap = 16384;
constexpr int kContribHdr = 128;
__host__ __device__ __forceinline__ int contrib_cap_for(int n_ranks) {
    return n_ranks <= 1 ? 8192 : (n_ranks == 2 ? 4096 : (n_ranks <= 4 ? 2048 : (n_ranks <= 8 ? 1024 : 512)));
}
__host__ __device__ __forceinline__ size_t contrib_floats(int cap) { return (size_t)kContribHdr + (size_t)cap * 32; }
constexpr int kAccRows = 64;
constexpr int kRec = 32;
__host__ __device__ __forceinline__ size_t band_at(int comp, size_t slot) { return slot * kRec + (size_t)comp; }

__device__ __forceinline__ void p2pl_products(float3 p, float4 q, float4 nn, float w, float* vals) {
    float F[6];
    float a = p.y * nn.z, b = p.z * nn.y;
    F[0] = a - b;
    a = p.z * nn.x; b = p.x * nn.z;
    F[1] = a - b;
    a = p.x * nn.y; b = p.y * nn.x;
    F[2] = a - b;
    F[3] = nn.x; F[4] = nn.y; F[5] = nn.z;
    const float dx = p.x - q.x, dy = p.y - q.y, dz = p.z - q.z;
    float r = dx * nn.x;
    float t2 = dy * nn.y;
    r = r + t2;
// ... 237 lines not shown
            float bb = nr.y * nt.y;
            float val = a + bb;
            a = nr.z * nt.z;
            val = val + a;
            if (val < f.cos_max_angle) w = 0.f;
        }
        cls = md2 < band_lo ? 0 : (md2 < band_hi ? 1 : 2);
        row[9] = 1.f;
        if (cls == 0) row[11] = 1.f;
        if (w != 0.f && cls == 0) {
            float a = p.y * nn.z, bq = p.z * nn.y;
            row[0] = a - bq;
            a = p.z * nn.x; bq = p.x * nn.z;
            row[1] = a - bq;
            a = p.x * nn.y; bq = p.y * nn.x;
            row[2] = a - bq;
            row[3] = nn.x; row[4] = nn.y; row[5] = nn.z;
            const float dx = p.x - tq.x, dy = p.y - tq.y, dz = p.z - tq.z;
            float r = dx * nn.x;
            float t2 = dy * nn.y;
            r = r + t2;
            t2 = dz * nn.z;
            r = r + t2;
            row[6] = r;
            row[7] = 1.f;
            row[8] = 1.f;
            row[10] = md2;
        }
        if (cls == 1) write_band_record(it, band, band_cap, p, tq, nn, w, md2, (int)q);
    }
    pos_io[q] = mpos;
    d2_out[q] = mpos >= 0 ? md2 : INFINITY;
    if (w_out) w_out[q] = (cls == 2) ? 0.f : w;
}

__device__ __forceinline__ double coh_component(const float* E, int rows, int comp) {
    double acc = 0.0;
    if (comp < 28) {
        const int ia = kProdCode.a[comp] >> 2, ic = kProdCode.c[comp] >> 2;
        for (int i = 0; i < rows; ++i) {
            const float v = E[i * kCohRow + ia] * E[i * kCohRow + ic];
            acc += (double)v;
        }
    } else {
        const int ia = 8 + (comp - 28);
        for (int i = 0; i < rows; ++i) acc += (double)E[i * kCohRow + ia];
    }
    return acc;
}

__global__ void __launch_bounds__(256)
k_coh_check(const float4* __restrict__ src, const float4* __restrict__ src_nrm, int64_t n, IterState* __restrict__ it,
            Grid g, const float4* __restrict__ tgt_nrm, FilterCfg f, int* __restrict__ pos_io, float* __restrict__ d2_out,
            float* __restrict__ w_out, const float4* __restrict__ cache ,
            uint32_t* __restrict__ queue, int queue_cap, float* __restrict__ band, int band_cap, double* __restrict__ partials,
            int n_blocks) {
    __shared__ __attribute__((aligned(16))) float E[256 * kCohRow];
    __shared__ int s_wave_cnt[4];
    __shared__ unsigned s_base;
    __shared__ double sh[4][kSums];
    const int t = threadIdx.x;
    const int lb = xcd_block(n_blocks);
    const int64_t q = lb < n_blocks ? (int64_t)lb * 256 + t : n;
    const int64_t qc = q < n ? q : n - 1;
    const float4 s = src[qc];
    const float4 c = cache[qc];
    const float4 tq = cache[(size_t)n + qc];
    const float4 nn = cache[2 * (size_t)n + qc];
    const float4 ru = cache[3 * (size_t)n + qc];
    const int pprev = pos_io[qc];
    const int st_done = it->done, st_stall = it->stall;
    const Xf T = load_xf(it);
    const float band_lo = it->band_lo, band_hi = it->band_hi;
    unsigned int* const qcount = it->qcount;
#pragma unroll
    for (int k = 0; k < 12; ++k) asm volatile("" ::"s"(T.m[k]));
    asm volatile("" ::"s"(band_lo), "s"(band_hi));
    asm volatile("" ::"v"(s.x), "v"(c.w), "v"(pprev), "v"(tq.x), "v"(nn.x), "v"(ru.x));
    if ((st_done | st_stall) != 0) return;
    const float3 p = xf_point(T, s.x, s.y, s.z);
    bool pass = false;
    float md2 = INFINITY;
    if (q < n && c.w > 0.f && pprev >= 0 && nn.w == 1.f) {
        const float dx = p.x - tq.x, dy = p.y - tq.y, dz = p.z - tq.z;
        float a = dx * dx;
        float b = dy * dy;
        float d2 = a + b;
        a = dz * dz;
        d2 = d2 + a;
        const float ex = p.x - c.x, ey = p.y - c.y, ez = p.z - c.z;
        const float delta = __builtin_amdgcn_sqrtf(ex * ex + ey * ey + ez * ez);
        const float lhs = (__builtin_amdgcn_sqrtf(d2) + delta) * 1.00001f + 1e-30f;
        const float rhs = __builtin_amdgcn_sqrtf(c.w) * 0.99999f;
        pass = d2 <= g.max_d2 && lhs < rhs;
        if (ru.w == 1.f) {
            const float fx = p.x - ru.x, fy = p.y - ru.y, fz = p.z - ru.z;
            float a2 = fx * fx;
            float b2 = fy * fy;
            float r2 = a2 + b2;
            a2 = fz * fz;
            r2 = r2 + a2;
            pass = pass && d2 < r2;
        }
        md2 = d2;
    }
    const bool need = q < n && !pass;
    const unsigned long long bal = __ballot(need);
    const int lane = t & 63, wave = t >> 6;
    if (lane == 0) s_wave_cnt[wave] = (int)__popcll(bal);
    __syncthreads();
    if (t == 0) {
        const int tot = s_wave_cnt[0] + s_wave_cnt[1] + s_wave_cnt[2] + s_wave_cnt[3];
        s_base = tot ? atomicAdd(&qcount[(lb & (kQueues - 1)) * kQueueStride], (unsigned)tot) : 0u;
    }
    __syncthreads();
    if (need) {
        unsigned at = s_base + (unsigned)__popcll(bal & ((1ull << lane) - 1ull));
        for (int w2 = 0; w2 < wave; ++w2) at += (unsigned)s_wave_cnt[w2];
        queue[(size_t)(lb & (kQueues - 1)) * queue_cap + at] = (uint32_t)q;
    }
    float row[12];
    if (pass) {
        coh_epilogue(T, f, band_lo, band_hi, p, q, pprev, md2, tq, nn, src_nrm, it, band, band_cap, pos_io, d2_out, w_out, row);
    } else {
#pragma unroll
        for (int k = 0; k < 12; ++k) row[k] = 0.f;
    }
#pragma unroll
    for (int k = 0; k < 12; ++k) E[t * kCohRow + k] = row[k];
    __syncthreads();
    const int comp = t & (kSums - 1), part = t >> 5;
    double acc = coh_component(E + (part * 32) * kCohRow, 32, comp);
    acc += __shfl_xor(acc, 32);
    if (lane < kSums) sh[wave][lane] = acc;
    __syncthreads();
    if (t < kSums && lb < n_blocks) {
        const double tot = (sh[0][t] + sh[1][t]) + (sh[2][t] + sh[3][t]);
        unsafeAtomicAdd(&partials[(size_t)(lb & (kAccRows - 1)) * kSums + t], tot);
    }
}

template <int G>
__global__ void __launch_bounds__(256, O3D_SEARCH_WAVES)
k_coh_search(const float4* __restrict__ src, const float4* __restrict__ src_nrm, int64_t n, IterState* __restrict__ it,
             Grid g, const float4* __restrict__ tgt_nrm, FilterCfg f, int* __restrict__ pos_io, float* __restrict__ d2_out,
             float* __restrict__ w_out, uint8_t* __restrict__ hint, float4* __restrict__ cache,
             const uint32_t* __restrict__ queue, int queue_cap, float* __restrict__ band, int band_cap,
             double* __restrict__ partials, float slack, CohStats* __restrict__ stats) {
    constexpr int kQ = 256 / G;
    __shared__ __attribute__((aligned(16))) uint32_t seg_lds[kQ * kSegWords<G>];
    __shared__ __attribute__((aligned(16))) float E[kQ * kCohRow];
    __shared__ double sh[4][kSums];
    __shared__ unsigned s_pre[kQueues + 1];
    const int t = threadIdx.x;
    const int st_done = it->done, st_stall = it->stall;
    const Xf T = load_xf(it);
    const float band_lo = it->band_lo, band_hi = it->band_hi;
    const unsigned int* const qcount = it->qcount;
    if ((st_done | st_stall) != 0) return;
    if (t < 64) {
        static_assert(kQueues == 64, "one lane per sub-queue");
        const unsigned cnt = qcount[t * kQueueStride];
        unsigned incl = cnt;
#pragma unroll
        for (int o = 1; o < 64; o <<= 1) {
            const unsigned v = (unsigned)__shfl_up((int)incl, o);
            if (t >= o) incl += v;
        }
        s_pre[t + 1] = incl;
        if (t == 0) s_pre[0] = 0u;
    }
    __syncthreads();
    const unsigned count = s_pre[kQueues];
    if ((unsigned)blockIdx.x * kQ >= count) return;
    const int sub = t & (G - 1), grp = t / G;
    const int comp = t & (kSums - 1), part = t >> 5;
    double acc = 0.0;
    for (unsigned base = (unsigned)blockIdx.x * kQ; base < count; base += gridDim.x * kQ) {
        const unsigned slot = base + (unsigned)grp;
        float row[12];
#pragma unroll
        for (int k = 0; k < 12; ++k) row[k] = 0.f;
        if (slot < count) {
            int sq = 0;
#pragma unroll
            for (int step = kQueues / 2; step >= 1; step >>= 1)
                if (s_pre[sq + step] <= slot) sq += step;
            const int64_t qq = (int64_t)queue[(size_t)sq * queue_cap + (slot - s_pre[sq])];
            const float4 s2 = src[qq];
            const int hv = hint ? (int)hint[qq] : 0;
            const float3 p2 = xf_point(T, s2.x, s2.y, s2.z);
            int lvl;
            float cov2;
            const Best bb = nearest_group<G, O3D_COH_PRUNE != 0, true>(g, p2, sub, -1, &lvl, seg_lds + grp * kSegWords<G>,
                                                          hv >= 2 ? hv - 2 : -1, &cov2, slack);
            if (sub == 0) {
                if (hint) hint[qq] = (uint8_t)(lvl + 1);
                const int pc = bb.pos >= 0 ? bb.pos : 0;
                const float4 tq = tgt_nrm[2 * (size_t)pc];
                float4 nn = tgt_nrm[2 * (size_t)pc + 1];
                nn.w = 1.f;
                float4 ru = make_float4(INFINITY, INFINITY, INFINITY, 1.f);
                if (bb.pos2 >= 0) {
                    const float4 t2 = g.pts[bb.pos2];
                    ru = make_float4(t2.x, t2.y, t2.z, 1.f);
                }
                cache[qq] = make_float4(p2.x, p2.y, p2.z, bb.pos >= 0 ? fminf(bb.third, cov2) : -1.f);
                cache[(size_t)n + qq] = tq;
                cache[2 * (size_t)n + qq] = nn;
                cache[3 * (size_t)n + qq] = ru;
                coh_epilogue(T, f, band_lo, band_hi, p2, qq, bb.pos, bb.d2, tq, nn, src_nrm, it, band, band_cap, pos_io, d2_out, w_out,
                             row);
            }
        }
        if (sub == 0) {
#pragma unroll
            for (int k = 0; k < 12; ++k) E[grp * kCohRow + k] = row[k];
        }
        __syncthreads();
        acc += coh_component(E + (part * (kQ / 8)) * kCohRow, kQ / 8, comp);
        __syncthreads();
    }
    acc += __shfl_xor(acc, 32);
    const int lane = t & 63, wave = t >> 6;
    if (lane < kSums) sh[wave][lane] = acc;
    __syncthreads();
    if (t < kSums) {
        const double tot = (sh[0][t] + sh[1][t]) + (sh[2][t] + sh[3][t]);
        unsafeAtomicAdd(&partials[(size_t)(blockIdx.x & (kAccRows - 1)) * kSums + t], tot);
    }
    if (stats && t == 0 && blockIdx.x == 0) {
        atomicAdd(&stats->n_points, (unsigned long long)n);
        atomicAdd(&stats->n_searched, (unsigned long long)count);
    }
}

__device__ __forceinline__ void block_pick1024(const uint32_t* h, int nb, uint32_t rank, uint32_t* wave_tot ,
                                               uint32_t* out ) {
    const int t = threadIdx.x;
    const uint32_t a = (2 * t < nb) ? h[2 * t] : 0u;
    const uint32_t b = (2 * t + 1 < nb) ? h[2 * t + 1] : 0u;
    const uint32_t sum = a + b;
    uint32_t incl = sum;
    const int lane = t & 63, wave = t >> 6;
    for (int o = 1; o < 64; o <<= 1) {
        const uint32_t v = __shfl_up(incl, o);
        if (lane >= o) incl += v;
    }
    if (lane == 63) wave_tot[wave] = incl;
    if (t == 0) {
        out[0] = 0;
        out[1] = 0;
    }
    __syncthreads();
    uint32_t base = 0;
    for (int w = 0; w < wave; ++w) base += wave_tot[w];
    const uint32_t excl = base + incl - sum;
    if (a && rank >= excl && rank < excl + a) {
        out[0] = 2 * t;
        out[1] = rank - excl;
    }
    if (b && rank >= excl + a && rank < excl + a + b) {
        out[0] = 2 * t + 1;
        out[1] = rank - excl - a;
    }
    __syncthreads();
}
```

### open3d_slam_private_amd/csrc/kernels_match.hpp

```cpp
#pragma once


__global__ void __launch_bounds__(256)
k_match(const float4* __restrict__ src, int64_t n, const IterState* __restrict__ it, Grid g, int* __restrict__ pos,
        float* __restrict__ d2, uint32_t* __restrict__ hist0 , uint32_t* __restrict__ hist2_to_zero,
        int shift0) {
    __shared__ uint32_t sh[2048];
    if (it->done) return;
    const Xf T = load_xf(it);
    if (hist2_to_zero && blockIdx.x == 0)
        for (int k = threadIdx.x; k < 2048; k += blockDim.x) hist2_to_zero[k] = 0;
    if (hist0) {
        for (int k = threadIdx.x; k < 2048; k += blockDim.x) sh[k] = 0;
        __syncthreads();
    }
    const int64_t i = blockIdx.x * (int64_t)blockDim.x + threadIdx.x;
    if (i < n) {
        const float4 s = src[i];
        const float3 p = xf_point(T, s.x, s.y, s.z);
        const Best b = nearest(g, p);
        pos[i] = b.pos;
        d2[i] = b.pos >= 0 ? b.d2 : INFINITY;
        if (hist0 && b.pos >= 0) atomicAdd(&sh[__float_as_uint(b.d2) >> shift0], 1u);
    }
    if (hist0) {
        __syncthreads();
        for (int k = threadIdx.x; k < 2048; k += blockDim.x)
            if (sh[k]) atomicAdd(&hist0[k], sh[k]);
    }
}

#ifndef O3D_MATCH_REGROUP
#define O3D_MATCH_REGROUP 1
#endif
template <int G>
constexpr int kSegWords = (2 * G * kSegPerLane + 2 + 3) & ~3;

template <int G>
__global__ void __launch_bounds__(256, O3D_MATCH_WAVES)
k_match_g8(const float4* __restrict__ src, int64_t n, const IterState* __restrict__ it, Grid g, int* __restrict__ pos,
           float* __restrict__ d2, uint32_t* __restrict__ hist0 ,
           uint32_t* __restrict__ hist2_to_zero, uint8_t* __restrict__ hint, int shift0, int debug, int n_blocks,
           float4* __restrict__ cache ,
           int xcd_tile ) {
    __shared__ uint32_t sh[2048];
    __shared__ __attribute__((aligned(16))) uint32_t seg_lds[(256 / G) * kSegWords<G>];
    const int lb = xcd_block_tiled(n_blocks, xcd_tile);
    const int64_t tid = lb * (int64_t)blockDim.x + threadIdx.x;
    const int64_t q = lb < n_blocks ? (tid / G) : n;
    const int sub = (int)(tid & (G - 1));
    const int64_t qc = q < n ? q : n - 1;
    const float4 s = src[qc];
    const uint8_t hraw = *(hint ? hint + qc : reinterpret_cast<const uint8_t*>(src));
    const int st_done = it->done;
    const Xf T = load_xf(it);
#pragma unroll
    for (int k = 0; k < 12; ++k) asm volatile("" ::"s"(T.m[k]));
    asm volatile("" ::"v"(s.x), "v"(s.y), "v"(s.z));
    if (st_done) return;
    if (hist2_to_zero && blockIdx.x == 0)
        for (int k = threadIdx.x; k < 2048; k += blockDim.x) hist2_to_zero[k] = 0;
    if (hist0) {
        for (int k = threadIdx.x; k < 2048; k += blockDim.x) sh[k] = 0;
        __syncthreads();
    }
    if (debug & 4) {
        if (q < n && sub == 0) {
            pos[q] = -1;
            d2[q] = xf_point(T, s.x, s.y, s.z).x;
        }
        return;
    }
    auto emit = [&](int64_t qq, const float3 pp, const Best& b, int lvl, float cov2) {
        pos[qq] = b.pos;
        d2[qq] = b.pos >= 0 ? b.d2 : INFINITY;
        if (hint) hint[qq] = (uint8_t)(lvl + 1);
        if (cache) {
            cache[qq] = make_float4(pp.x, pp.y, pp.z, b.pos >= 0 ? fminf(b.second, cov2) : -1.f);
            cache[3 * (size_t)n + qq] = make_float4(0.f, 0.f, 0.f, 0.f);
        }
        if (hist0 && b.pos >= 0) atomicAdd(&sh[__float_as_uint(b.d2) >> shift0], 1u);
    };
    constexpr int kP = 256 / G;
    constexpr int kKeys = 2 * kMaxLevels + 2;
    __shared__ float4 un_p[kP], un_b[kP];
    __shared__ uint32_t un_l[kP];
    __shared__ uint32_t key_cnt[kKeys + 1];
    const int grp = (int)(threadIdx.x / G);
    const int gbase = (int)(threadIdx.x & 63) & ~(G - 1);
    for (int k = threadIdx.x; k <= kKeys; k += blockDim.x) key_cnt[k] = 0u;
    __syncthreads();
    const float3 p = xf_point(T, s.x, s.y, s.z);
    Best b;
    float cov = 0.f, cov2 = 0.f;
    int l = 0, lvl = 0, key = -1;
    uint32_t rnk = 0;
    if (q < n) {
        const int hv = hint ? (int)hraw : 0;
        if (nearest_halo<G, false, true>(g, p, sub, gbase, -1, hv >= 2 ? hv - 2 : -1, b, cov, l, &lvl, &cov2)) {
            if (sub == 0) emit(q, p, b, lvl, cov2);
#if !O3D_MATCH_REGROUP
        } else if (true) {
            b = nearest_levels<G, true, false>(g, p, sub, gbase, l, b, cov, seg_lds + grp * kSegWords<G>, 0.f, &lvl, &cov2);
            if (sub == 0) emit(q, p, b, lvl, cov2);
#endif
        } else {
            key = min(l, kMaxLevels) + (b.pos >= 0 ? 0 : kMaxLevels + 1);
            if (sub == 0) rnk = atomicAdd(&key_cnt[key], 1u);
            rnk = (uint32_t)__shfl((int)rnk, gbase);
        }
    }
    __syncthreads();
    if (threadIdx.x < 64) {
        const uint32_t c = (int)threadIdx.x < kKeys ? key_cnt[threadIdx.x] : 0u;
        uint32_t incl = c;
#pragma unroll
        for (int o = 1; o < 64; o <<= 1) {
            const uint32_t v = (uint32_t)__shfl_up((int)incl, o);
            if ((int)threadIdx.x >= o) incl += v;
        }
        if ((int)threadIdx.x < kKeys) key_cnt[threadIdx.x] = incl - c;
        if (threadIdx.x == kKeys - 1) key_cnt[kKeys] = incl;
    }
    __syncthreads();
    if (key >= 0 && sub == 0) {
        const uint32_t at = key_cnt[key] + rnk;
        un_p[at] = make_float4(p.x, p.y, p.z, cov);
        un_b[at] = make_float4(b.d2, __uint_as_float(b.idx), __int_as_float(b.pos), b.second);
        un_l[at] = (uint32_t)l | ((uint32_t)grp << 8);
    }
    __syncthreads();
    if (grp < (int)key_cnt[kKeys]) {
        const float4 ep = un_p[grp], eb = un_b[grp];
        const uint32_t el = un_l[grp];
        const int64_t q2 = (int64_t)lb * kP + (int64_t)(el >> 8);
        const float3 p2 = make_float3(ep.x, ep.y, ep.z);
        Best b2;
        b2.d2 = eb.x;
        b2.idx = __float_as_uint(eb.y);
        b2.pos = __float_as_int(eb.z);
        b2.second = eb.w;
        b2.pos2 = -1;
        b2.third = INFINITY;
        b2 = nearest_levels<G, true, false>(g, p2, sub, gbase, (int)(el & 255u), b2, ep.w, seg_lds + grp * kSegWords<G>, 0.f, &lvl, &cov2);
        if (sub == 0) emit(q2, p2, b2, lvl, cov2);
    }
    if (hist0) {
        __syncthreads();
        for (int k = threadIdx.x; k < 2048; k += blockDim.x)
            if (sh[k]) atomicAdd(&hist0[k], sh[k]);
    }
}

struct SelectState {
    uint32_t prefix;
    uint32_t rank;
    uint32_t n_finite;
    uint32_t done;
    float limit;
    uint32_t pad[3];
};


__device__ __forceinline__ void block_pick256_regs(const uint32_t (&loc)[8], uint32_t rank, uint32_t* wave_tot ,
                                                   uint32_t* out ) {
    const int t = threadIdx.x;
    uint32_t sum = 0;
#pragma unroll
    for (int k = 0; k < 8; ++k) sum += loc[k];
    uint32_t incl = sum;
    const int lane = t & 63, wave = t >> 6;
    for (int o = 1; o < 64; o <<= 1) {
        const uint32_t v = __shfl_up(incl, o);
        if (lane >= o) incl += v;
    }
    if (lane == 63) wave_tot[wave] = incl;
    if (t == 0) {
        out[0] = 0;
        out[1] = 0;
    }
    __syncthreads();
    uint32_t base = 0, total = 0;
#pragma unroll
    for (int w = 0; w < 4; ++w) {
        const uint32_t v = wave_tot[w];
        if (w < wave) base += v;
        total += v;
    }
    if (t == 0) out[2] = total;
    uint32_t run = base + incl - sum;
#pragma unroll
    for (int k = 0; k < 8; ++k) {
        if (loc[k] && rank >= run && rank < run + loc[k]) {
            out[0] = (uint32_t)(t * 8 + k);
            out[1] = rank - run;
        }
        run += loc[k];
    }
    __syncthreads();
}

__device__ __forceinline__ void load_hist8(const uint32_t* __restrict__ hist, uint32_t (&loc)[8]) {
    const uint4 a = reinterpret_cast<const uint4*>(hist)[threadIdx.x * 2];
    const uint4 b = reinterpret_cast<const uint4*>(hist)[threadIdx.x * 2 + 1];
    loc[0] = a.x; loc[1] = a.y; loc[2] = a.z; loc[3] = a.w;
    loc[4] = b.x; loc[5] = b.y; loc[6] = b.z; loc[7] = b.w;
}

__device__ __forceinline__ void block_pick256(const uint32_t* __restrict__ hist, int nb, uint32_t rank,
                                              uint32_t* wave_tot , uint32_t* out ) {
    uint32_t loc[8];
#pragma unroll
    for (int k = 0; k < 8; ++k) {
        const int bin = threadIdx.x * 8 + k;
        loc[k] = bin < nb ? hist[bin] : 0u;
    }
    block_pick256_regs(loc, rank, wave_tot, out);
}

__device__ __forceinline__ uint32_t trim_rank(uint32_t total, float ratio) {
    if (total == 0) return 0;
    if (ratio == 1.0f) return total - 1;
    const float posf = (float)total * ratio;
    uint32_t r = (uint32_t)posf;
    return r >= total ? total - 1 : r;
}

// ... 475 lines not shown
```

### open3d_slam_private_amd/csrc/kernels_tail.hpp

```cpp
#pragma once

#ifndef O3D_TAIL_ACQ
#define O3D_TAIL_ACQ 0
#endif
#ifndef O3D_TAIL_THREADS
#define O3D_TAIL_THREADS 512
#endif
constexpr int kTailThreads = O3D_TAIL_THREADS;
#ifndef O3D_TAIL_SLOTS
#define O3D_TAIL_SLOTS 1024
#endif
#ifndef O3D_TAIL_WGS_PER_CU
#define O3D_TAIL_WGS_PER_CU 1
#endif
constexpr int kTailSlots = O3D_TAIL_SLOTS;
constexpr int kTailWgsPerCu = O3D_TAIL_WGS_PER_CU;
constexpr int kTailPts = kTailSlots / kTailThreads;
constexpr int kTailRec = 12;
constexpr int kTailHistRow = 32;
constexpr int kTailCoarse = 256;
constexpr int kTailMaxIters = 64;
constexpr int kTailSyncWords = 256;
constexpr int kTailRing = 4;
constexpr int kTailBandCntWord = 128;
constexpr int kTailAccRows = 16;
constexpr int kTailAccDoubles = kTailRing * kTailAccRows * kSums;
constexpr int kTailSyncBytes = kTailSyncWords * 4 + kTailAccDoubles * 8;
constexpr int kTailArriveStride = 16;
constexpr int kTailErrWord = 192;
constexpr int kTailSearchedWord = 193;
constexpr int kTailItersWord = 194;
constexpr int kTailCauseWord = 195;
constexpr int kTailStampWord = 200;
constexpr int kTailGroups = kTailThreads / 8;
constexpr int kTailBins = 1024;
#ifndef O3D_TAIL_STAMPS
#define O3D_TAIL_STAMPS 0
#endif
#ifndef O3D_TAIL_G4
#define O3D_TAIL_G4 0
#endif
#if O3D_TAIL_STAMPS
#define TAIL_STAMP(i)                                                      \
    do {                                                                   \
        const unsigned long long now_ = __builtin_amdgcn_s_memrealtime();  \
        stamp_acc[i] += now_ - stamp_last;                                 \
        stamp_last = now_;                                                 \
    } while (0)
#else
#define TAIL_STAMP(i) do { } while (0)
#endif

struct TailCfg {
    int64_t n;
    int chunk8;
    int wpc;
    int tile;
    int max_iters;
    float slack;
    unsigned long long seq;
    unsigned long long timeout_ticks;
};

struct TailLds {
    static constexpr int kRows = 0;
    static constexpr int kUnion = kRows + 5 * kTailSlots * 16;
    static constexpr int kUnionSeg = (kTailThreads / 8) * kSegWords<8> * 4, kUnionSeg4 = O3D_TAIL_G4 ? (kTailThreads / 4) * kSegWords<4> * 4 : 0;
    static constexpr int kUnionMax = kUnionSeg > kUnionSeg4 ? (kUnionSeg > kTailBandCap * 8 ? kUnionSeg : kTailBandCap * 8)
                                                            : (kUnionSeg4 > kTailBandCap * 8 ? kUnionSeg4 : kTailBandCap * 8);
    static constexpr int kUnionBytes = (kUnionMax + 255) & ~255;
    static constexpr int kD2 = kUnion + kUnionBytes;
    static constexpr int kFail = kD2 + kTailSlots * 4;
    static constexpr int kWcls = kFail + kTailSlots * 2;
    static constexpr int kHint = kWcls + kTailSlots;
    static constexpr int kSh = kHint + kTailSlots;
    static constexpr int kTot = kSh + 16 * kSums * 8;
    static constexpr int kState = kTot + kSums * 8;
    static constexpr int kStateBytes = (int)((sizeof(IterState) + 15) & ~size_t(15));
    static constexpr int kMisc = kState + kStateBytes;
    static constexpr int kWtot = kMisc + 64;
    static constexpr int kOff = kWtot + 64;
    static constexpr int kX = kOff + 272 * 4;
    static constexpr int kWork = kX + 96;
    static constexpr int kMirror = kWork + kUpdWorkBytes;
    static constexpr int kMirrorBytes = (int)((sizeof(HostMirror) + 15) & ~size_t(15));
    static constexpr int kHist = kMirror + kMirrorBytes;
    static constexpr int kTotal = kHist + kTailBins * 4;
    static constexpr int kBk = kUnion;
};
static_assert(TailLds::kBk + kTailBandCap * 8 - TailLds::kUnion <= TailLds::kUnionBytes, "phase-C scratch exceeds the union");
static_assert(kTailGroups * kSegWords<8> * 4 <= TailLds::kUnionBytes, "segment lists exceed the union");
static_assert(TailLds::kTotal * kTailWgsPerCu <= 160 * 1024, "LDS budget of one CU");
constexpr int kTailLdsBytes = TailLds::kTotal;

__device__ __forceinline__ double tail_ld_f64(const double* p) {
    const unsigned long long v = __hip_atomic_load(reinterpret_cast<unsigned long long*>(const_cast<double*>(p)), __ATOMIC_RELAXED,
                                                   __HIP_MEMORY_SCOPE_AGENT);
    return __longlong_as_double((long long)v);
}
__device__ __forceinline__ void tail_st_f64(double* p, double x) {
    __hip_atomic_store(reinterpret_cast<unsigned long long*>(p), (unsigned long long)__double_as_longlong(x), __ATOMIC_RELAXED,
                       __HIP_MEMORY_SCOPE_AGENT);
}
__device__ __forceinline__ unsigned long long tail_ld_u64(const void* p) {
    return __hip_atomic_load(reinterpret_cast<unsigned long long*>(const_cast<void*>(p)), __ATOMIC_RELAXED, __HIP_MEMORY_SCOPE_AGENT);
}
__device__ __forceinline__ void tail_st_u64(void* p, unsigned long long x) {
    __hip_atomic_store(reinterpret_cast<unsigned long long*>(p), x, __ATOMIC_RELAXED, __HIP_MEMORY_SCOPE_AGENT);
}
__device__ __forceinline__ unsigned tail_ld_u32(const unsigned* p) {
    return __hip_atomic_load(const_cast<unsigned*>(p), __ATOMIC_RELAXED, __HIP_MEMORY_SCOPE_AGENT);
}

__device__ __noinline__ __attribute__((flatten)) void tail_solve_update(IterState* sit, const double* tot, const uint32_t* misc, float* s_x, UpdWork* work,
                                               bool trim, unsigned n_band_raw, unsigned n_band_all) {
    const int lane = (int)(threadIdx.x & 63);
    const float r_limit_last = sit->limit_last, r_limit_sel = __uint_as_float(misc[2]);
    const int r_dbg_narrow = sit->debug_narrow_band & 1;
    const int r_fixed = sit->fixed_iters, r_iters = sit->iterations;
    const int r_xnc = sit->xicp_nc;
    const double r_tot28 = tot[28];
    float r_T[16];
#pragma unroll
    for (int i = 0; i < 16; ++i) r_T[i] = sit->T[i];
    const int r = lane >> 3, c = lane & 7;
    double a = 0.0;
    if (r < 6 && c < 7) {
        if (c < 6) {
            const int lo = r < c ? r : c, hi = r < c ? c : r;
            const int k = lo * 6 - (lo * (lo - 1)) / 2 + (hi - lo);
            a = (double)(float)tot[k];
        } else {
            a = (double)(-(float)tot[21 + r]);
        }
    }
    const double a_orig = a;
    double dmax = 0.0;
#pragma unroll
    for (int j = 0; j < 6; ++j) dmax = fmax(dmax, fabs(__shfl(a_orig, j * 8 + j)));
    bool well = dmax > 0.0;
    const double piv_thr = 1e-4 * dmax;
#pragma unroll
// ... 251 lines not shown
    unsigned long long* const bk = reinterpret_cast<unsigned long long*>(lds + TailLds::kBk);
    float* const d2s = reinterpret_cast<float*>(lds + TailLds::kD2);
    uint16_t* const fail = reinterpret_cast<uint16_t*>(lds + TailLds::kFail);
    uint8_t* const wcls = reinterpret_cast<uint8_t*>(lds + TailLds::kWcls);
    uint8_t* const hnt = reinterpret_cast<uint8_t*>(lds + TailLds::kHint);
    double (*const sh)[kSums] = reinterpret_cast<double (*)[kSums]>(lds + TailLds::kSh);
    double* const tot = reinterpret_cast<double*>(lds + TailLds::kTot);
    uint32_t* const s_state = reinterpret_cast<uint32_t*>(lds + TailLds::kState);
    IterState* const sit = reinterpret_cast<IterState*>(s_state);
    uint32_t* const misc = reinterpret_cast<uint32_t*>(lds + TailLds::kMisc);
    uint32_t* const wtot = reinterpret_cast<uint32_t*>(lds + TailLds::kWtot);
    uint32_t* const off = reinterpret_cast<uint32_t*>(lds + TailLds::kOff);
    float* const s_x = reinterpret_cast<float*>(lds + TailLds::kX);
    UpdWork* const work = reinterpret_cast<UpdWork*>(lds + TailLds::kWork);
    uint32_t* const mir_w = reinterpret_cast<uint32_t*>(lds + TailLds::kMirror);
    uint32_t* const hist = reinterpret_cast<uint32_t*>(lds + TailLds::kHist);
    double* const acc_g = reinterpret_cast<double*>(sync + kTailSyncWords);
    constexpr int kStateWords = (int)(sizeof(IterState) / 4);
    constexpr int kWaves = kTailThreads / 64;
    static_assert(kStateWords <= kTailThreads && kTailThreads >= 256, "state staging / count scan by the first threads");

    const int t = threadIdx.x, lane = t & 63, wave = t >> 6;
    const int nwg = (int)gridDim.x;
    const int xcls = (int)(blockIdx.x & 7), wq = (int)(blockIdx.x >> 3);
    const int64_t n = cfg.n;
    int64_t q[kTailPts];
    bool valid[kTailPts];
    float4 s[kTailPts], sn[kTailPts];
    float4 sc1[kTailPts];
#pragma unroll
    for (int u = 0; u < kTailPts; ++u) {
        const int sl = t + u * kTailThreads;
        const int64_t oc = (int64_t)(sl >> 3) * cfg.wpc + wq;
        const int64_t r_in = oc * 8 + (sl & 7);
        if (cfg.tile > 0) {
            const int64_t tl = oc / cfg.tile, rr = oc - tl * cfg.tile;
            q[u] = ((tl * 8 + xcls) * cfg.tile + rr) * 8 + (sl & 7);
        } else {
            q[u] = (int64_t)xcls * cfg.chunk8 + r_in;
        }
        valid[u] = r_in < cfg.chunk8 && q[u] < n;
        if (!valid[u]) q[u] = 0;
    }
    if (t < kStateWords) s_state[t] = reinterpret_cast<const uint32_t*>(it_g)[t];
#pragma unroll
    for (int u = 0; u < kTailPts; ++u) {
        const int sl = t + u * kTailThreads;
        float4 r0 = cache[q[u]], r1 = cache[(size_t)n + q[u]];
        const float4 r2 = cache[2 * (size_t)n + q[u]], r3 = cache[3 * (size_t)n + q[u]];
        const int pprev = pos_io[q[u]];
        s[u] = src[q[u]];
        sc1[u] = make_float4(0.f, 0.f, 0.f, 0.f);
        if (kGicp) {
            sn[u] = src_nrm[2 * q[u]];
            sc1[u] = src_nrm[2 * q[u] + 1];
            const int pc = pprev >= 0 ? pprev : 0;
            r1 = g.pts[pc];
            float4 c0 = tgt_nrm[2 * (size_t)pc], c1 = tgt_nrm[2 * (size_t)pc + 1];
            c1.w = (valid[u] && pprev >= 0) ? 1.f : 0.f;
            st_rows[2 * kTailSlots + sl] = c0;
            st_rows[4 * kTailSlots + sl] = c1;
        } else {
            sn[u] = f.use_normal ? src_nrm[q[u]] : make_float4(0.f, 0.f, 0.f, 0.f);
            st_rows[2 * kTailSlots + sl] = r2;
        }
        if (!valid[u]) r0.w = -1.f;
        r1.w = __int_as_float(valid[u] ? pprev : -1);
        st_rows[sl] = r0;
        st_rows[kTailSlots + sl] = r1;
        st_rows[3 * kTailSlots + sl] = r3;
        hnt[sl] = hint_g ? hint_g[q[u]] : (uint8_t)0;
        d2s[sl] = INFINITY;
        wcls[sl] = 0;
    }
    for (int k = t; k < kTailBins; k += kTailThreads) hist[k] = 0u;
    if (t < 16) misc[t] = 0u;
    __syncthreads();
    if (sit->done || sit->stall) {
        if (blockIdx.x == 0)
            for (int w2 = t; w2 < kTailSyncBytes / 4; w2 += kTailThreads) sync_next[w2] = 0u;
        return;
    }
    const unsigned cnt_lane = lane < 8 ? (unsigned)((nwg - lane + 7) >> 3) : 0u;
    unsigned n_searched = 0;
    int exit_reason = 0;
    int k_local = 0;
    unsigned epoch = 0;
#if O3D_TAIL_STAMPS
    unsigned long long stamp_acc[12] = {0, 0, 0, 0, 0, 0, 0, 0, 0, 0, 0, 0};
    unsigned long long stamp_last = __builtin_amdgcn_s_memrealtime();
#endif
    int tv = t;

    auto exchange = [&](unsigned set) -> bool {
        if (blockIdx.x == 0) {
            const unsigned nxt = (epoch + 2u) & (kTailRing - 1);
            if (t < kTailAccRows * kSums) tail_st_f64(acc_g + (size_t)nxt * kTailAccRows * kSums + tv, 0.0);
            if (t == 0) __hip_atomic_store(&sync[kTailBandCntWord + 16 * nxt], 0u, __ATOMIC_RELAXED, __HIP_MEMORY_SCOPE_AGENT);
        }
        asm volatile("s_waitcnt vmcnt(0)" ::: "memory");
        __syncthreads();
        ++epoch;
        if (wave == 0) {
            if (lane < kSums) {
                double v = 0.0;
#pragma unroll
                for (int w2 = 0; w2 < kWaves; ++w2) v += sh[w2][lane];
                const int row = (int)(blockIdx.x & 7) * (kTailAccRows / 8) + (int)((blockIdx.x >> 3) & (kTailAccRows / 8 - 1));
                unsafeAtomicAdd(acc_g + ((size_t)set * kTailAccRows + row) * kSums + lane, v);
            }
            asm volatile("s_waitcnt vmcnt(0)" ::: "memory");
            if (lane == 0) __hip_atomic_fetch_add(&sync[xcls * kTailArriveStride], 1u, __ATOMIC_RELAXED, __HIP_MEMORY_SCOPE_AGENT);
            const unsigned target = epoch * cnt_lane;
            const unsigned long long t0 = __builtin_amdgcn_s_memrealtime();
            bool okp = false;
            for (;;) {
                const unsigned v = lane < 8 ? tail_ld_u32(&sync[lane * kTailArriveStride]) : 0u;
                okp = __all(lane >= 8 || v >= target) != 0;
                if (okp) break;
                __builtin_amdgcn_s_sleep(1);
                if (__builtin_amdgcn_s_memrealtime() - t0 > cfg.timeout_ticks) break;
            }
#if O3D_TAIL_ACQ
            __builtin_amdgcn_fence(__ATOMIC_ACQUIRE, "agent");
            asm volatile("s_waitcnt vmcnt(0)" ::: "memory");
#endif
            if (lane == 0) misc[3] = okp ? 1u : 0u;
        }
        __syncthreads();
        return misc[3] != 0u;
    };
    auto publish_sums = [&](double (&v)[kSums]) {
        wave_reduce32(v);
        if ((lane & 1) == 0) sh[wave][lane >> 1] = v[0];
    };
    auto reduce_sums = [&](unsigned set, bool add) {
        static_assert(kTailAccRows * kSums == kTailThreads, "one accumulator entry per thread");
        double a = tail_ld_f64(acc_g + (size_t)set * kTailAccRows * kSums + tv);
        a += __shfl_xor(a, 32);
        if (lane < kSums) sh[wave][lane] = a;
        __syncthreads();
        if (t < kSums) {
            double v = 0.0;
#pragma unroll
            for (int w2 = 0; w2 < kWaves; ++w2) v += sh[w2][t];
            tot[t] = add ? tot[t] + v : v;
        }
        __syncthreads();
    };
    auto accumulate = [&](double (&v)[kSums], const float (&F)[7], float md2) {
        int k = 0;
#pragma unroll
        for (int a6 = 0; a6 < 6; ++a6)
#pragma unroll
            for (int c6 = a6; c6 < 6; ++c6) v[k++] += (double)(F[a6] * F[c6]);
#pragma unroll
        for (int a6 = 0; a6 < 6; ++a6) v[21 + a6] += (double)(F[a6] * F[6]);
        v[27] += (double)(F[6] * F[6]);
        v[28] += 1.0;
        v[30] += (double)md2;
    };
    auto reserve_records = [&](unsigned set, const bool (&mine)[kTailPts], unsigned (&slot)[kTailPts]) {
        unsigned long long bal[kTailPts];
        unsigned nw = 0;
#pragma unroll
        for (int u = 0; u < kTailPts; ++u) {
            bal[u] = __ballot(mine[u]);
            nw += (unsigned)__popcll(bal[u]);
        }
        unsigned base = 0;
        if (nw != 0u) {
            if (lane == 0) base = atomicAdd(&sync[kTailBandCntWord + 16 * set], nw);
            base = (unsigned)__shfl((int)base, 0);
        }
        unsigned before = 0;
#pragma unroll
        for (int u = 0; u < kTailPts; ++u) {
            slot[u] = base + before + (unsigned)__popcll(bal[u] & ((1ull << lane) - 1ull));
            before += (unsigned)__popcll(bal[u]);
        }
    };
    auto store_record = [&](int buf, unsigned slotb, const float (&F)[7], float md2, float w) {
        if (slotb >= (unsigned)kTailBandCap) return;
        float* rec = band_g + ((size_t)buf * kTailBandCap + slotb) * kTailRec;
        const float kept = w != 0.f ? 1.f : 0.f;
        const float v[12] = {F[0], F[1], F[2], F[3], F[4], F[5], F[6], md2, kept, 0.f, w != 0.f ? md2 : 0.f, 0.f};
#pragma unroll
        for (int k = 0; k < 6; ++k)
            tail_st_u64(rec + 2 * k, ((unsigned long long)__float_as_uint(v[2 * k + 1]) << 32) | __float_as_uint(v[2 * k]));
    };

    for (;; ++k_local) {
        tv = t;
        asm volatile("" : "+v"(tv));
        Xf T;
#pragma unroll
        for (int k = 0; k < 12; ++k) T.m[k] = __int_as_float(__builtin_amdgcn_readfirstlane(__float_as_int(sit->T[k])));
        const float band_lo = sit->band_lo, band_hi = sit->band_hi;
        const bool trim = !kGicp && sit->use_trim && sit->trim_ratio != 1.0f;
        const bool wide = trim && band_hi < INFINITY && (band_hi - band_lo) > kTailWideRel * band_lo;
        const uint32_t u_lo = __float_as_uint(band_lo), u_hi = __float_as_uint(band_hi);
        const double f_scale = (wide ? (double)kTailCoarse : 1.0) / (double)(u_hi > u_lo ? u_hi - u_lo : 1u);
        auto coarse_bin = [&](float d2) -> uint32_t {
            return min((uint32_t)((double)(__float_as_uint(d2) - u_lo) * f_scale), (uint32_t)(kTailCoarse - 1));
        };
        float3 p[kTailPts];
#pragma unroll
        for (int u = 0; u < kTailPts; ++u) {
            const int sl = t + u * kTailThreads;
            p[u] = xf_point(T, s[u].x, s[u].y, s[u].z);
            const float4 c = st_rows[sl], tq = st_rows[kTailSlots + sl], nn = st_rows[2 * kTailSlots + sl],
                         ru = st_rows[3 * kTailSlots + sl];
            const int pprev = __float_as_int(tq.w);
            bool pass = false;
            const float attr_ok = kGicp ? st_rows[4 * kTailSlots + sl].w : nn.w;
            if (valid[u] && c.w > 0.f && pprev >= 0 && attr_ok == 1.f) {
                const float dx = p[u].x - tq.x, dy = p[u].y - tq.y, dz = p[u].z - tq.z;
                float a = dx * dx;
                float b2 = dy * dy;
                float d2 = a + b2;
                a = dz * dz;
                d2 = d2 + a;
                const float ex = p[u].x - c.x, ey = p[u].y - c.y, ez = p[u].z - c.z;
                const float delta = __builtin_amdgcn_sqrtf(ex * ex + ey * ey + ez * ez);
                const float lhs = (__builtin_amdgcn_sqrtf(d2) + delta) * 1.00001f + 1e-30f;
                const float rhs = __builtin_amdgcn_sqrtf(c.w) * 0.99999f;
                pass = d2 <= g.max_d2 && lhs < rhs;
                if (ru.w == 1.f) {
                    const float fx = p[u].x - ru.x, fy = p[u].y - ru.y, fz = p[u].z - ru.z;
                    float a2 = fx * fx;
                    float b3 = fy * fy;
                    float r2 = a2 + b3;
                    a2 = fz * fz;
                    r2 = r2 + a2;
                    pass = pass && d2 < r2;
                }
                if (pass) d2s[sl] = d2;
            }
            if (valid[u] && !pass) {
                const unsigned at = atomicAdd(&misc[0], 1u);
                fail[at] = (uint16_t)sl;
                st_rows[sl] = make_float4(p[u].x, p[u].y, p[u].z, -1.f);
            }
        }
        __syncthreads();
        TAIL_STAMP(0);
        const int nf = (int)misc[0];
        n_searched += (t == 0) ? (unsigned)nf : 0u;
        auto search_rounds = [&](auto gtag) {
            constexpr int G = decltype(gtag)::value;
            constexpr int kGroups = kTailThreads / G;
            const int sub = t & (G - 1), grp = t / G;
            for (int base = 0; base < nf; base += kGroups) {
                const int fi = base + grp;
                if (fi < nf) {
                    const int slot = (int)fail[fi];
                    const float4 a0 = st_rows[slot];
                    const float3 p2 = make_float3(a0.x, a0.y, a0.z);
                    const int hv = (int)hnt[slot];
                    int lvl;
                    float cov2;
                    const Best bb = nearest_group<G, O3D_COH_PRUNE != 0, true>(g, p2, sub, -1, &lvl, seg_lds + grp * kSegWords<G>,
                                                                               hv >= 2 ? hv - 2 : -1, &cov2, cfg.slack);
                    if (sub == 0) {
                        hnt[slot] = (uint8_t)(lvl + 1);
                        st_rows[slot] = make_float4(p2.x, p2.y, p2.z, bb.pos >= 0 ? fminf(bb.third, cov2) : -1.f);
                        st_rows[kTailSlots + slot].w = __int_as_float(bb.pos);
                        st_rows[3 * kTailSlots + slot].w = __int_as_float(bb.pos2);
                        d2s[slot] = bb.pos >= 0 ? bb.d2 : INFINITY;
                    }
                }
            }
        };
#if O3D_TAIL_G4
        if (nf > kTailThreads / 8)
            search_rounds(std::integral_constant<int, 4>());
        else
#endif
            search_rounds(std::integral_constant<int, 8>());
        __syncthreads();
#pragma unroll 1
        for (int fi = tv; fi < nf; fi += kTailThreads) {
            const int slot = (int)fail[fi];
            const int pos = __float_as_int(st_rows[kTailSlots + slot].w), pos2 = __float_as_int(st_rows[3 * kTailSlots + slot].w);
            const size_t pc = (size_t)(pos >= 0 ? pos : 0), pc2 = (size_t)(pos2 >= 0 ? pos2 : 0);
            const float4 t2 = g.pts[pc2];
            float4 tq = kGicp ? g.pts[pc] : tgt_nrm[2 * pc];
            float4 nn = kGicp ? tgt_nrm[2 * pc] : tgt_nrm[2 * pc + 1];
            if (kGicp) {
                float4 c1 = tgt_nrm[2 * pc + 1];
                c1.w = 1.f;
                st_rows[4 * kTailSlots + slot] = c1;
            } else {
                nn.w = 1.f;
            }
            tq.w = __int_as_float(pos);
            st_rows[kTailSlots + slot] = tq;
            st_rows[2 * kTailSlots + slot] = nn;
            st_rows[3 * kTailSlots + slot] = pos2 >= 0 ? make_float4(t2.x, t2.y, t2.z, 1.f)
                                                       : make_float4(INFINITY, INFINITY, INFINITY, 1.f);
        }
        __syncthreads();
        TAIL_STAMP(1);
        float rF[kTailPts][7], md2v[kTailPts], wv[kTailPts];
        int clsv[kTailPts];
        const unsigned set = epoch & (kTailRing - 1);
        int buf = (int)(epoch & 1u);
        {
            double v[kSums];
#pragma unroll
            for (int k = 0; k < kSums; ++k) v[k] = 0.0;
#pragma unroll
            for (int u = 0; u < kTailPts; ++u) {
                const int sl = t + u * kTailThreads;
#pragma unroll
                for (int k = 0; k < 7; ++k) rF[u][k] = 0.f;
                const float4 tq = st_rows[kTailSlots + sl], nn = st_rows[2 * kTailSlots + sl];
                const int mpos = valid[u] ? __float_as_int(tq.w) : -1;
                const float md2 = d2s[sl];
                float w = 0.f;
                int cls = 2;
                if (kGicp) {
                    if (valid[u] && mpos >= 0) {
                        w = 1.f;
                        cls = 0;
                        tail_gicp_factor(T, s[u], sn[u], sc1[u], tq, nn, st_rows[4 * kTailSlots + sl], md2, v);
                    }
                } else if (valid[u] && mpos >= 0) {
                    w = 1.f;
                    if (f.use_maxdist && !(md2 <= f.outlier_max_d2)) w = 0.f;
                    if (f.use_normal) {
                        const float3 nr = normalize3(xf_rot(T, sn[u].x, sn[u].y, sn[u].z));
                        const float3 nt = normalize3(make_float3(nn.x, nn.y, nn.z));
                        float a = nr.x * nt.x;
                        float bb2 = nr.y * nt.y;
                        float val = a + bb2;
                        a = nr.z * nt.z;
                        val = val + a;
                        if (val < f.cos_max_angle) w = 0.f;
                    }
                    cls = md2 < band_lo ? 0 : (md2 < band_hi ? 1 : 2);
                    if (w != 0.f && cls != 2) {
                        float a = p[u].y * nn.z, bq = p[u].z * nn.y;
                        rF[u][0] = a - bq;
                        a = p[u].z * nn.x; bq = p[u].x * nn.z;
                        rF[u][1] = a - bq;
                        a = p[u].x * nn.y; bq = p[u].y * nn.x;
                        rF[u][2] = a - bq;
                        rF[u][3] = nn.x; rF[u][4] = nn.y; rF[u][5] = nn.z;
                        const float dx = p[u].x - tq.x, dy = p[u].y - tq.y, dz = p[u].z - tq.z;
                        float r = dx * nn.x;
                        float t2 = dy * nn.y;
                        r = r + t2;
                        t2 = dz * nn.z;
                        r = r + t2;
                        rF[u][6] = r;
                    }
                    v[29] += 1.0;
                    if (cls == 0) v[31] += 1.0;
                    if (w != 0.f && cls == 0) accumulate(v, rF[u], md2);
                }
                if (!(valid[u] && mpos >= 0)) d2s[sl] = INFINITY;
                wcls[sl] = (uint8_t)((w != 0.f && cls != 2 ? 1 : 0) | (cls << 1));
                md2v[u] = md2;
                wv[u] = w;
                clsv[u] = cls;
                if (wide && cls == 1) atomicAdd(&hist[coarse_bin(md2)], 1u);
            }
            unsigned slot[kTailPts];
            if (!wide) {
                bool mine[kTailPts];
#pragma unroll
                for (int u = 0; u < kTailPts; ++u) mine[u] = clsv[u] == 1;
                reserve_records(set, mine, slot);
            }
            publish_sums(v);
            if (!wide) {
#pragma unroll
                for (int u = 0; u < kTailPts; ++u)
                    if (clsv[u] == 1) store_record(buf, slot[u], rF[u], md2v[u], wv[u]);
            }
        }
        TAIL_STAMP(2);
        if (wide) {
            __syncthreads();
            if (t < kTailCoarse / 8) {
                unsigned long long pk = 0ull;
#pragma unroll
                for (int j = 0; j < 8; ++j) {
                    const uint32_t c2 = hist[8 * t + j];
                    hist[8 * t + j] = 0u;
                    pk |= (unsigned long long)min(c2, 255u) << (8 * j);
                }
                tail_st_u64(hist_g + ((size_t)buf * nwg + blockIdx.x) * kTailHistRow + tv, pk);
            }
        }
        if (t == 0) {
            misc[0] = 0u;
            misc[5] = 0u;
            misc[9] = 0u;
            misc[2] = __float_as_uint(INFINITY);
        }
        TAIL_STAMP(3);
        if (!exchange(set)) {
            exit_reason = 4;
            if (t == 0) __hip_atomic_fetch_add(&sync[kTailErrWord], 1u, __ATOMIC_RELAXED, __HIP_MEMORY_SCOPE_AGENT);
            break;
        }
        TAIL_STAMP(5);
        uint32_t sel_bin = 0;
        bool stall = false;
        unsigned rset = set;
        unsigned long long rv[6] = {0ull, 0ull, 0ull, 0ull, 0ull, 0ull};
        unsigned n_band_raw = 0;
        auto load_records_spec = [&]() {
            n_band_raw = tail_ld_u32(&sync[kTailBandCntWord + 16 * rset]);
            const float* rec = band_g + ((size_t)buf * kTailBandCap + (unsigned)tv) * kTailRec;
#pragma unroll
            for (int k = 0; k < 6; ++k) rv[k] = tail_ld_u64(rec + 2 * k);
        };
        if (!wide) load_records_spec();
        reduce_sums(set, false);
        TAIL_STAMP(6);
        if (trim && wide && (uint32_t)llround(tot[29]) != 0u) {
            {
                const unsigned* wbase = reinterpret_cast<const unsigned*>(hist_g + (size_t)buf * nwg * kTailHistRow) + (tv & 63);
                constexpr int kG = kTailThreads / 64, kL = (256 * kTailWgsPerCu) / kG;
                unsigned c4[4] = {0, 0, 0, 0};
                bool sat = false;
                for (int u0 = 0; u0 < kL; u0 += 8) {
                    unsigned wv2[8];
#pragma unroll
                    for (int u = 0; u < 8; ++u) {
                        const int b2 = (tv >> 6) + kG * (u0 + u);
                        wv2[u] = b2 < nwg ? tail_ld_u32(wbase + (size_t)b2 * (kTailHistRow * 2)) : 0u;
                    }
#pragma unroll
                    for (int u = 0; u < 8; ++u)
#pragma unroll
                        for (int j = 0; j < 4; ++j) {
                            const unsigned bv = (wv2[u] >> (8 * j)) & 255u;
                            sat = sat || bv == 255u;
                            c4[j] += bv;
                        }
                }
                if (sat) misc[5] = 1u;
#pragma unroll
                for (int j = 0; j < 4; ++j)
                    if (c4[j]) atomicAdd(&hist[4 * (t & 63) + j], c4[j]);
            }
            __syncthreads();
            const uint32_t n_finite = (uint32_t)llround(tot[29]), n_below = (uint32_t)llround(tot[31]);
            const uint32_t kq = trim_rank(n_finite, sit->trim_ratio);
            if (t < 256) {
                const uint32_t hv2 = hist[t];
                hist[t] = 0u;
                uint32_t incl = hv2;
#pragma unroll
                for (int o = 1; o < 64; o <<= 1) {
                    const uint32_t v = (uint32_t)__shfl_up((int)incl, o);
                    if (lane >= o) incl += v;
                }
                if (lane == 63) wtot[wave] = incl;
                off[t] = incl - hv2;
            }
            __syncthreads();
            if (t < 256) {
                uint32_t base = 0;
#pragma unroll
                for (int w2 = 0; w2 < 4; ++w2) base += w2 < wave ? wtot[w2] : 0u;
                off[t] += base;
                if (t == 0) misc[12] = wtot[0] + wtot[1] + wtot[2] + wtot[3];
            }
            __syncthreads();
            {
                const uint32_t total_band = misc[12];
                if (!(n_below <= kq && kq < n_below + total_band) || misc[5] != 0u) stall = true;
                if (!stall && t < 256) {
                    const uint32_t excl = off[t], nxt = t == 255 ? total_band : off[t + 1];
                    const uint32_t rank = kq - n_below;
                    if (nxt > excl && rank >= excl && rank < nxt) misc[10] = (uint32_t)t;
// ... 120 lines not shown
#pragma unroll
                for (int u = 0; u < kTailPts; ++u) {
                    const unsigned i = (unsigned)(t + u * kTailThreads);
                    const unsigned long long* r6 = u == 0 ? rv : rv2;
                    const float d2r = __uint_as_float((unsigned)(r6[3] >> 32)), keptr = __uint_as_float((unsigned)r6[4]);
                    if (i < n_band && d2r <= limit && keptr != 0.f) {
                        const float F[7] = {__uint_as_float((unsigned)r6[0]), __uint_as_float((unsigned)(r6[0] >> 32)),
                                            __uint_as_float((unsigned)r6[1]), __uint_as_float((unsigned)(r6[1] >> 32)),
                                            __uint_as_float((unsigned)r6[2]), __uint_as_float((unsigned)(r6[2] >> 32)),
                                            __uint_as_float((unsigned)r6[3])};
                        accumulate(v, F, d2r);
                    }
                }
                wave_reduce32(v);
                if ((lane & 1) == 0) sh[wave][lane >> 1] = v[0];
                __syncthreads();
                if (t < kSums) {
                    double v2 = 0.0;
#pragma unroll
                    for (int w2 = 0; w2 < kWaves; ++w2) v2 += sh[w2][t];
                    tot[t] += v2;
                }
                __syncthreads();
            }
        }
        TAIL_STAMP(10);
        if (t < kSums) sit->sums[t] = tot[t];
        if (wave == 0) {
            if (kGicp)
                tail_solve_update_gicp(sit, tot, reinterpret_cast<double*>(s_x), work);
            else
                tail_solve_update(sit, tot, misc, s_x, work, trim, n_band_raw, wide ? misc[12] : n_band_raw);
        }
        __syncthreads();
        TAIL_STAMP(11);
        if (sit->done) {
            exit_reason = 1;
            ++k_local;
            break;
        }
        if (k_local + 1 >= cfg.max_iters) {
            exit_reason = 3;
            ++k_local;
            break;
        }
    }
    if (exit_reason == 2 || exit_reason == 4) {
        if (t == 0) {
            sit->stall = 1;
            sit->band_count = 0;
        }
        __syncthreads();
    }
#pragma unroll
    for (int u = 0; u < kTailPts; ++u) {
        if (!valid[u]) continue;
        const int sl = t + u * kTailThreads;
        const float4 tq = st_rows[kTailSlots + sl];
        const int cls = (int)(wcls[sl] >> 1);
        float w = (wcls[sl] & 1) ? 1.f : 0.f;
        if (cls == 1 && !(d2s[sl] <= __uint_as_float(misc[2]))) w = 0.f;
        pos_io[q[u]] = __float_as_int(tq.w);
        d2_out[q[u]] = d2s[sl];
        if (w_out) w_out[q[u]] = w;
        if (hint_g) hint_g[q[u]] = hnt[sl];
    }
    if (exit_reason == 3) {
        for (int sl = t; sl < kTailSlots; sl += kTailThreads) {
            const int64_t oc = (int64_t)(sl >> 3) * cfg.wpc + wq;
            const int64_t r_in = oc * 8 + (sl & 7);
            int64_t qq;
            if (cfg.tile > 0) {
                const int64_t tl = oc / cfg.tile, rr = oc - tl * cfg.tile;
                qq = ((tl * 8 + xcls) * cfg.tile + rr) * 8 + (sl & 7);
            } else {
                qq = (int64_t)xcls * cfg.chunk8 + r_in;
            }
            if (r_in < cfg.chunk8 && qq < n) {
#pragma unroll
                for (int r = 0; r < 4; ++r) cache[(size_t)r * (size_t)n + qq] = st_rows[r * kTailSlots + sl];
            }
        }
    }
    if (t == 0 && n_searched) atomicAdd(&sync[kTailSearchedWord], n_searched);
#if O3D_TAIL_STAMPS
    if (t == 0 && (blockIdx.x == 0 || blockIdx.x == gridDim.x - 1)) {
        unsigned long long* out = reinterpret_cast<unsigned long long*>(sync + kTailStampWord) + (blockIdx.x == 0 ? 0 : 12);
        for (int i = 0; i < 12; ++i) out[i] = stamp_acc[i];
    }
#endif
    if (blockIdx.x != 0) return;
    for (int w2 = t; w2 < kTailSyncBytes / 4; w2 += kTailThreads) sync_next[w2] = 0u;
    if (t == 0) sync[kTailItersWord] = (unsigned)k_local;
    if (wave != 0) return;
    if (lane == 0) {
        HostMirror* m = reinterpret_cast<HostMirror*>(mir_w);
        for (int i = 0; i < 16; ++i) m->T[i] = sit->T[i];
        for (int i = 0; i < 16; ++i) m->T_prev[i] = sit->T_prev[i];
        m->iterations = sit->iterations;
        m->done = sit->done;
        m->status = exit_reason == 4 ? (int)REG_DEVICE_ERROR : sit->status;
        m->rank_last = sit->rank_last;
        m->converged = sit->chk.converged ? 1 : 0;
        m->max_iter_reached = sit->chk.max_iter_reached ? 1 : 0;
        m->stall = sit->stall;
        m->band_count = (int)sit->band_count;
        m->limit_last = sit->limit_last;
        m->limit_prev = sit->limit_prev;
        m->band_lo = sit->band_lo;
        m->band_hi = sit->band_hi;
        m->pad_nband = (int)sit->band_count;
        m->pad2 = exit_reason;
        for (int i = 0; i < 6; ++i) {
            m->localizable[i] = sit->xicp_flags[i];
            m->xicp_comb[i] = sit->xicp_comb[i];
            m->xicp_high[i] = sit->xicp_high[i];
        }
        m->n_constraints = sit->xicp_nc;
        m->pad3 = k_local;
        for (int i = 0; i < 8; ++i) m->stamps[i] = 0ull;
        if (sit->stall == 0) sit->band_count = 0;
    }
    if (lane < kSums) reinterpret_cast<HostMirror*>(mir_w)->sums[lane] = sit->sums[lane];
    __builtin_amdgcn_fence(__ATOMIC_ACQ_REL, "workgroup");
    __builtin_amdgcn_wave_barrier();
    for (int w2 = lane; w2 < kStateWords; w2 += 64) reinterpret_cast<uint32_t*>(it_g)[w2] = s_state[w2];
    constexpr int kMirrorWords = (int)(offsetof(HostMirror, seq) / 4);
    uint32_t* hw = reinterpret_cast<uint32_t*>(host);
    for (int w2 = lane; w2 < kMirrorWords; w2 += 64) hw[w2] = mir_w[w2];
    HostMirror::SeqRecord* srec = &host->ring[cfg.seq % kSeqRing];
    {
        const HostMirror* m = reinterpret_cast<const HostMirror*>(mir_w);
        uint32_t word = 0;
        if (lane == 2) word = (uint32_t)m->iterations;
        if (lane == 3) word = (uint32_t)m->done;
        if (lane == 4) word = (uint32_t)m->stall;
        if (lane == 6) word = __float_as_uint(m->limit_last);
        if (lane == 7) word = __float_as_uint(m->limit_prev);
        if (lane >= 2 && lane < 8) reinterpret_cast<uint32_t*>(srec)[lane] = word;
    }
    __threadfence_system();
    if (lane == 0) {
        __hip_atomic_store(&srec->seq, cfg.seq, __ATOMIC_RELEASE, __HIP_MEMORY_SCOPE_SYSTEM);
        __hip_atomic_store(&host->seq, cfg.seq, __ATOMIC_RELEASE, __HIP_MEMORY_SCOPE_SYSTEM);
    }
}
```

### open3d_slam_private_amd/csrc/reg_state.hpp

```cpp
#pragma once

struct IterState {
    float T[16];
    float T_prev[16];
    double Td[16];
    Checkers chk;
    int iterations;
    int done;
    int status;
    int rank_last;
    int cost;
    int fixed_iters;
    int max_iter;
    int update;
    float gicp_rot_eps, gicp_trans_eps;
    int gicp_stop_rule;
    float gicp_rel_fitness, gicp_rel_rmse;
    float n_total;
    double fit_prev, rmse_prev;
    double sums[kSums];
    float band_lo, band_hi;
    float trim_ratio;
    int use_trim;
    int stall;
    float limit_last;
    float limit_prev;
    unsigned int band_count;
    unsigned int* qcount;
    unsigned int band_cap;
    int debug_narrow_band;
    float limit_prev2;
    int xicp_stage;
    int xicp_nc;
    int xicp_flags[6];
    float xicp_enough, xicp_insufficient, xicp_cos_min, xicp_cos_strong;
    float xicp_Trd[12];
    double xicp_comb[6], xicp_high[6];
};

struct XicpState {
    float vr[9], vt[9];
    int pad[2];
    double center[4];
    double comb[6], high[6];
};

struct HostMirror {
    double sums[kSums];
    float T[16];
    float T_prev[16];
    int iterations, done, status, rank_last, converged, max_iter_reached, stall, band_count;
    float limit_last, limit_prev, band_lo, band_hi;
    int pad_nband, pad2;
    int localizable[6];
    int n_constraints, pad3;
    double xicp_comb[6], xicp_high[6];
    unsigned long long stamps[8];
    unsigned long long seq;
    struct SeqRecord {
        unsigned long long seq;
        int iterations, done, stall, pad;
        float limit_last, limit_prev;
    } ring[16];
};
constexpr int kSeqRing = 16;

constexpr int kTailBandCap = 1024;
constexpr float kTailWideRel = 0.02f;
constexpr float kBandFloor = 0.003f;
constexpr float kBandRatioMax = 0.6f;
constexpr float kBandCentreGain = 1.5f;
constexpr float kBandGeomRel = 0.25f;
constexpr float kBandGuardFrac = 0.75f;
constexpr float kBandForcedWide = 0.0205f;
struct Band {
    float lo, hi;
};
__host__ __device__ inline Band predict_band(float limit, float prev, float prev2, unsigned last_count, float last_lo, float last_hi,
                                             int debug_narrow) {
    Band b = {INFINITY, INFINITY};
    if (!(limit < INFINITY)) return b;
    float m = 0.3f;
    if (prev < INFINITY && prev > 0.f) m = fminf(fmaxf(2.0f * fabsf(limit - prev) / limit + kBandFloor, kBandFloor), 0.6f);
    if (debug_narrow) m = 1e-7f;
    b.lo = limit * (1.0f - m);
    b.hi = limit * (1.0f + m);
    if (debug_narrow) return b;
    if (prev < INFINITY && prev > 0.f && prev2 < INFINITY && prev2 > 0.f) {
        const float d = limit - prev, dp = prev - prev2;
        if (d * dp > 0.f && fabsf(d) < fabsf(dp) && fabsf(dp) <= kBandGeomRel * limit) {
            const float q = d / dp;
            const float far_edge = limit + fmaxf(kBandCentreGain * q, kBandRatioMax) * d, pad = kBandFloor * limit;
            b.lo = d < 0.f ? far_edge - pad : limit - pad;
            b.hi = d < 0.f ? limit + pad : far_edge + pad;
        }
    }
    if (last_count > 0u && last_hi < INFINITY && last_hi > last_lo) {
        const float est = (float)last_count * (b.hi - b.lo) / (last_hi - last_lo);
        if (est > kBandGuardFrac * (float)kTailBandCap && !(b.hi - b.lo > kTailWideRel * b.lo)) {
            const float grow = 0.5f * (kBandForcedWide * limit - (b.hi - b.lo));
            if (grow > 0.f) {
                b.lo -= grow;
                b.hi += grow;
            }
        }
    }
    return b;
}
constexpr int kQueues = 64;
constexpr int kQueueStride = 16;

__device__ __forceinline__ int xcd_block(int n_blocks) {
    const int chunk = (n_blocks + 7) >> 3;
    return (int)(blockIdx.x & 7) * chunk + (int)(blockIdx.x >> 3);
}

__host__ __device__ __forceinline__ int xcd_tiled_grid(int n_blocks, int tile) {
    if (tile <= 0) return 8 * ((n_blocks + 7) / 8);
    const int per = 8 * tile;
    return per * ((n_blocks + per - 1) / per);
}
__device__ __forceinline__ int xcd_block_tiled(int n_blocks, int tile) {
    if (tile <= 0) return xcd_block(n_blocks);
    const int xcd = (int)(blockIdx.x & 7), j = (int)(blockIdx.x >> 3);
    const int t = j / tile, r = j - t * tile;
    return (t * 8 + xcd) * tile + r;
}

struct Xf4 {
    float m[16];
};

__device__ __forceinline__ Xf load_xf(const IterState* it) {
    Xf x;
#pragma unroll
    for (int k = 0; k < 12; ++k) x.m[k] = it->T[k];
    return x;
}
```

Baseline: 19040.

## Add runner-up swap shortcut in tail and top-2 tracking in late match launches

Centralizes the coherent-shortcut test into a shared rule. The rule can now also swap to the cached runner-up neighbour when that neighbour provably becomes nearest, instead of falling back to a full nearest-neighbour search. The generic match kernel gains a top-2 variant for late launches, so the cache holds a runner-up for the following tail iterations. This adds extra work to tracking and swap handling in exchange for fewer full searches, and adds debug counters.

Measured after the change: 19130 (median of 6 runs). Within noise of the previous version (+0.5%).

```diff
diff --git a/include/o3dslam_reg_debug.h b/include/o3dslam_reg_debug.h
--- a/include/o3dslam_reg_debug.h
+++ b/include/o3dslam_reg_debug.h
@@ -26,6 +26,8 @@
 
 REG_API reg_status reg_debug_live_resources(int64_t out[4]);
 
+REG_API reg_status reg_debug_shortcut_counts(reg_handle* h, int64_t out[4]);
+
 #ifdef __cplusplus
 }
 #endif
diff --git a/open3d_slam_private_amd/capi.py b/open3d_slam_private_amd/capi.py
--- a/open3d_slam_private_amd/capi.py
+++ b/open3d_slam_private_amd/capi.py
@@ -382,7 +382,7 @@
            "reg_set_target_f64", "reg_get_target_source_indices", "reg_voxelize_within_volume", "reg_carve_indices", "reg_dist_xicp_buffers", "reg_dist_gather_buffers",
            "reg_dist_record", "reg_dist_centroid_sums", "reg_dist_prepare",
            "reg_information_matrix", "reg_set_source_f64", "reg_debug_configure", "reg_debug_halo_bound", "reg_debug_halo_witness",
-           "reg_debug_live_resources",
+           "reg_debug_live_resources", "reg_debug_shortcut_counts",
            "reg_dist_get_unique_id", "reg_dist_init", "reg_dist_init_custom", "reg_dist_register", "reg_dist_shutdown",
            "reg_dist_info", "reg_dist_steer_create", "reg_dist_steer_destroy", "reg_dist_steer_step",
            "reg_dist_steer_counts", "reg_host_tail_plan", "reg_host_o3d_update",
@@ -440,6 +440,7 @@
     lib.reg_debug_halo_bound.argtypes = [vp, f32p, i64, f32p]
     lib.reg_debug_halo_witness.argtypes = [vp, f32p, i64, vp]
     lib.reg_debug_live_resources.argtypes = [C.POINTER(C.c_int64)]
+    lib.reg_debug_shortcut_counts.argtypes = [vp, C.POINTER(C.c_int64)]
     lib.reg_dist_get_unique_id.argtypes = [C.c_char_p]
     lib.reg_dist_init.argtypes = [vp, C.c_char_p, C.c_int, C.c_int]
     lib.reg_dist_init_custom.argtypes = [vp, C.POINTER(Collectives), C.c_int, C.c_int]
@@ -1478,6 +1479,11 @@
         self._check(self._lib.reg_debug_halo_witness(self._h, _ptr(x), x.shape[0], _ptr(out)))
         return out
 
+    def shortcut_counts(self):
+        out = (C.c_int64 * 4)()
+        self._check(self._lib.reg_debug_shortcut_counts(self._h, out))
+        return tuple(int(v) for v in out)
+
     def prepare(self, T_init=None):
         Ti = _T_in(np.eye(4) if T_init is None else T_init)
         self._check(self._lib.reg_prepare(self._h, _ptr(Ti)))
@@ -1897,6 +1903,22 @@
     return np.float32(out[0]), np.float32(out[1])
 
 
+SHORTCUT_SEARCH, SHORTCUT_KEEP, SHORTCUT_SWAP = 0, 1, 2
+RUNNER_NONE, RUNNER_OFF = -1, -2
+
+
+def host_shortcut(p, anchor, g2, winner, runner, rpos, max_d2, allow_swap=True):
+    lib = load_library()
+    f3 = C.c_float * 3
+    lib.reg_host_shortcut.argtypes = [f3, C.c_float * 4, f3, f3, C.c_int32, C.c_float, C.c_int32, C.POINTER(C.c_float)]
+    lib.reg_host_shortcut.restype = C.c_int32
+    d2 = C.c_float(0.0)
+    a4 = (C.c_float * 4)(float(anchor[0]), float(anchor[1]), float(anchor[2]), float(g2))
+    out = lib.reg_host_shortcut(f3(*[float(v) for v in p]), a4, f3(*[float(v) for v in winner]), f3(*[float(v) for v in runner]),
+                                int(rpos), float(max_d2), 1 if allow_swap else 0, C.byref(d2))
+    return int(out), np.float32(d2.value)
+
+
 def host_band_constants():
     lib = load_library()
     lib.reg_host_predict_band.argtypes = [C.c_float, C.c_float, C.c_float, C.c_uint32, C.c_float, C.c_float, C.c_int32,
diff --git a/open3d_slam_private_amd/csrc/host_handle.hpp b/open3d_slam_private_amd/csrc/host_handle.hpp
--- a/open3d_slam_private_amd/csrc/host_handle.hpp
+++ b/open3d_slam_private_amd/csrc/host_handle.hpp
@@ -7,6 +7,8 @@
     bool no_dynprune = false;
     bool no_empty_bound = false;
     bool no_witness = false;
+    bool no_swap = false;
+    bool no_match_top2 = false;
     bool no_burst = false;
     bool hints = false;
     bool stamps = false;
@@ -40,6 +42,8 @@
         no_dynprune = getenv("O3D_NO_DYNPRUNE") != nullptr;
         no_empty_bound = getenv("O3D_NO_EMPTY_BOUND") != nullptr;
         no_witness = getenv("O3D_NO_WITNESS") != nullptr;
+        no_swap = getenv("O3D_NO_SWAP") != nullptr;
+        no_match_top2 = getenv("O3D_NO_MATCH_TOP2") != nullptr;
         halo_occ = getenv("O3D_NO_HALO_OCC") == nullptr;
         hints = getenv("O3D_HINTS") != nullptr;
         stamps = getenv("O3D_STAMPS") != nullptr;
@@ -142,9 +146,11 @@
     int last_stalls = 0;
     int64_t n_total_hint = 0;
     int match_launches = 0;
+    bool match_top2 = false;
     int tail_sync_slot = 0, tail_sync_last = 0;
     bool tail_sync_dirty = true;
     int last_tail_launches = 0, last_tail_iters = 0;
+    unsigned long long last_coh_points = 0, last_coh_searched = 0;
     DevBuf i_tail_sync, i_tail_rows, i_tail_band;
     unsigned long long dist_seq0 = 0;
     DevBuf d_contrib, d_gathered;
diff --git a/open3d_slam_private_amd/csrc/host_loop.hpp b/open3d_slam_private_amd/csrc/host_loop.hpp
--- a/open3d_slam_private_amd/csrc/host_loop.hpp
+++ b/open3d_slam_private_amd/csrc/host_loop.hpp
@@ -169,6 +169,8 @@
         const int lanes = h->dbg.lanes_per_point == 4 ? 4 : (h->dbg.lanes_per_point == 2 ? 2 : 8);
         const int blocks = grid_for(h->n * lanes);
         const int tile = h->match_launches < 2 ? h->env.xcd_tile_first : h->env.xcd_tile_later;
+        const bool top2 = h->match_top2 && h->match_launches >= 2 && !h->env.no_match_top2 && !cost_is_o3d(h->prm.cost);
+        h->match_top2 = false;
         ++h->match_launches;
         const dim3 grid(xcd_tiled_grid(blocks, tile)), block(256);
         auto go = [&](auto kernel) {
@@ -180,6 +182,8 @@
             go(k_match_g8<4>);
         else if (lanes == 2)
             go(k_match_g8<2>);
+        else if (top2)
+            go(k_match_g8<8, true>);
         else
             go(k_match_g8<8>);
     }
@@ -334,6 +338,7 @@
     cfg.tile = pl.tile;
     cfg.max_iters = std::max(1, std::min(max_iters, kTailMaxIters));
     cfg.slack = coherent_slack(h);
+    cfg.swap = h->env.no_swap ? 0 : 1;
     cfg.seq = ++h->seq;
     cfg.timeout_ticks = (unsigned long long)(h->env.tail_timeout_s * 1e8);
     uint8_t* hint = h->dbg.match_variant == 2 ? nullptr : h->i_hint.as<uint8_t>();
@@ -568,7 +573,7 @@
     }
     const bool reported = mirror_seq(h) >= tail_seq;
     const unsigned* sync_last = h->i_tail_sync.as<unsigned>() + (size_t)h->tail_sync_last * (kTailSyncBytes / 4);
-    unsigned words[4] = {0, 0, 0, 0};
+    unsigned words[5] = {0, 0, 0, 0, 0};
     if (!reported || h->env.coh_stats || mir->status == REG_DEVICE_ERROR)
         (void)hipMemcpy(words, sync_last + kTailErrWord, sizeof(words), hipMemcpyDeviceToHost);
     if (words[0] != 0 || (reported && mir->status == REG_DEVICE_ERROR)) {
@@ -579,8 +584,9 @@
     }
     if (!reported && !(mir->stall && std::max(mirror_seq(h), la.seq0) > la.acked)) la.acked = h->seq;
     if (h->env.coh_stats)
-        fprintf(stderr, "[o3dreg] tail launch: %u iterations, %u point searches (%.2f %% of the point-iterations), stall cause %u, band records of its last iteration %d\n", words[2],
-                words[1], words[2] ? 100.0 * words[1] / ((double)words[2] * (double)h->n) : 0.0, words[3], reported ? mir->pad_nband : -1);
+        fprintf(stderr, "[o3dreg] tail launch: %u iterations, %u point searches (%.2f %% of the point-iterations), %u swaps (%.2f %%), stall cause %u, band records of its last iteration %d\n", words[2],
+                words[1], words[2] ? 100.0 * words[1] / ((double)words[2] * (double)h->n) : 0.0, words[4],
+                words[2] ? 100.0 * words[4] / ((double)words[2] * (double)h->n) : 0.0, words[3], reported ? mir->pad_nband : -1);
     if (reported) h->last_tail_iters += mir->pad3;
     if (reported && mir->stall && h->prm.fixed_iters <= 0) *tail_off = true;
 #if O3D_TAIL_STAMPS
@@ -630,6 +636,8 @@
         if (hipMemcpy(&cs, h->i_stats.p, sizeof(cs), hipMemcpyDeviceToHost) == hipSuccess) {
             fprintf(stderr, "[o3dreg] coherent fused iterations: %llu point-iterations, %llu searched (%.2f %%)\n", cs.n_points,
                     cs.n_searched, cs.n_points ? 100.0 * (double)cs.n_searched / (double)cs.n_points : 0.0);
+            h->last_coh_points = cs.n_points;
+            h->last_coh_searched = cs.n_searched;
             (void)hipMemset(h->i_stats.p, 0, sizeof(cs));
         }
     }
@@ -677,6 +685,29 @@
                             kBandForcedWide};
         for (int i = 0; i < 8; ++i) consts[i] = c[i];
     }
+}
+
+REG_API int32_t reg_host_shortcut(const float p[3], const float anchor_g2[4], const float winner[3], const float runner[3],
+                                  int32_t rpos, float max_d2, int32_t allow_swap, float* d2_out) {
+    const Shortcut s = shortcut_rule(p[0], p[1], p[2], anchor_g2[0], anchor_g2[1], anchor_g2[2], anchor_g2[3], winner[0], winner[1],
+                                     winner[2], runner[0], runner[1], runner[2], rpos, max_d2, allow_swap != 0);
+    if (d2_out) *d2_out = s.outcome == kShortcutSearch ? INFINITY : s.d2;
+    return s.outcome;
+}
+
+reg_status reg_debug_shortcut_counts(reg_handle* h, int64_t out[4]) {
+    if (!h || !out) return REG_BAD_ARGUMENT;
+    if (!h->device_ok) return REG_DEVICE_ERROR;
+    HIPCHK(h, hipSetDevice(h->prm.device));
+    unsigned long long c[2] = {0, 0};
+    HIPCHK(h, hipMemcpy(c, reinterpret_cast<const char*>(h->i_iter.p) + offsetof(IterState, tail_searched), sizeof(c), hipMemcpyDeviceToHost));
+    const int64_t tested = (int64_t)h->last_tail_iters * h->n + (int64_t)h->last_coh_points;
+    const int64_t searched = (int64_t)c[0] + (int64_t)h->last_coh_searched, swapped = (int64_t)c[1];
+    out[0] = tested;
+    out[1] = tested - swapped - searched;
+    out[2] = swapped;
+    out[3] = searched;
+    return REG_OK;
 }
 
 reg_status reg_prepare(reg_handle* h, const float T_init[16]) {
@@ -768,6 +799,7 @@
     const auto t_loop0 = std::chrono::steady_clock::now();
     unsigned long long tail_seq = 0;
     h->last_stalls = h->last_tail_launches = h->last_tail_iters = 0;
+    h->last_coh_points = h->last_coh_searched = 0;
     for (;;) {
         if (tail_seq) {
             s = wait_tail(h, tail_seq, la, &pol.tail_off);
@@ -799,6 +831,9 @@
             const SteerChoice c = steer_choose(seen, pol);
             const auto tq0 = std::chrono::steady_clock::now();
             if (c.kind == SteerChoice::kGeneric) {
+                h->match_top2 = pol.use_tail && !pol.tail_off && la.completed + la.inflight + 1 >= pol.tail_min_iters && seen.any &&
+                                seen.step_trans <= pol.settle_trans && seen.step_rot <= pol.settle_rot &&
+                                (!pol.trimming || (seen.limit_prev < INFINITY && seen.limit_last < INFINITY));
                 s = enqueue_iteration(h, true);
                 if (generic_left > 0) --generic_left;
             } else if (c.kind == SteerChoice::kTail) {
diff --git a/open3d_slam_private_amd/csrc/kernels_fused.hpp b/open3d_slam_private_amd/csrc/kernels_fused.hpp
--- a/open3d_slam_private_amd/csrc/kernels_fused.hpp
+++ b/open3d_slam_private_amd/csrc/kernels_fused.hpp
@@ -343,27 +343,10 @@
     bool pass = false;
     float md2 = INFINITY;
     if (q < n && c.w > 0.f && pprev >= 0 && nn.w == 1.f) {
-        const float dx = p.x - tq.x, dy = p.y - tq.y, dz = p.z - tq.z;
-        float a = dx * dx;
-        float b = dy * dy;
-        float d2 = a + b;
-        a = dz * dz;
-        d2 = d2 + a;
-        const float ex = p.x - c.x, ey = p.y - c.y, ez = p.z - c.z;
-        const float delta = __builtin_amdgcn_sqrtf(ex * ex + ey * ey + ez * ez);
-        const float lhs = (__builtin_amdgcn_sqrtf(d2) + delta) * 1.00001f + 1e-30f;
-        const float rhs = __builtin_amdgcn_sqrtf(c.w) * 0.99999f;
-        pass = d2 <= g.max_d2 && lhs < rhs;
-        if (ru.w == 1.f) {
-            const float fx = p.x - ru.x, fy = p.y - ru.y, fz = p.z - ru.z;
-            float a2 = fx * fx;
-            float b2 = fy * fy;
-            float r2 = a2 + b2;
-            a2 = fz * fz;
-            r2 = r2 + a2;
-            pass = pass && d2 < r2;
-        }
-        md2 = d2;
+        const Shortcut sc = shortcut_rule(p.x, p.y, p.z, c.x, c.y, c.z, c.w, tq.x, tq.y, tq.z, ru.x, ru.y, ru.z, __float_as_int(ru.w),
+                                          g.max_d2, false);
+        pass = sc.outcome == kShortcutKeep;
+        if (pass) md2 = sc.d2;
     }
     const bool need = q < n && !pass;
     const unsigned long long bal = __ballot(need);
@@ -461,10 +444,10 @@
                 const float4 tq = tgt_nrm[2 * (size_t)pc];
                 float4 nn = tgt_nrm[2 * (size_t)pc + 1];
                 nn.w = 1.f;
-                float4 ru = make_float4(INFINITY, INFINITY, INFINITY, 1.f);
+                float4 ru = make_float4(INFINITY, INFINITY, INFINITY, __int_as_float(kRunnerNone));
                 if (bb.pos2 >= 0) {
                     const float4 t2 = g.pts[bb.pos2];
-                    ru = make_float4(t2.x, t2.y, t2.z, 1.f);
+                    ru = make_float4(t2.x, t2.y, t2.z, __int_as_float(bb.pos2));
                 }
                 cache[qq] = make_float4(p2.x, p2.y, p2.z, bb.pos >= 0 ? fminf(bb.third, cov2) : -1.f);
                 cache[(size_t)n + qq] = tq;
diff --git a/open3d_slam_private_amd/csrc/kernels_match.hpp b/open3d_slam_private_amd/csrc/kernels_match.hpp
--- a/open3d_slam_private_amd/csrc/kernels_match.hpp
+++ b/open3d_slam_private_amd/csrc/kernels_match.hpp
@@ -36,7 +36,7 @@
 template <int G>
 constexpr int kSegWords = (2 * G * kSegPerLane + 2 + 3) & ~3;
 
-template <int G>
+template <int G, bool kTop2 = false>
 __global__ void __launch_bounds__(256, O3D_MATCH_WAVES)
 k_match_g8(const float4* __restrict__ src, int64_t n, const IterState* __restrict__ it, Grid g, int* __restrict__ pos,
            float* __restrict__ d2, uint32_t* __restrict__ hist0 ,
@@ -76,14 +76,25 @@
         d2[qq] = b.pos >= 0 ? b.d2 : INFINITY;
         if (hint) hint[qq] = (uint8_t)(lvl + 1);
         if (cache) {
-            cache[qq] = make_float4(pp.x, pp.y, pp.z, b.pos >= 0 ? fminf(b.second, cov2) : -1.f);
-            cache[3 * (size_t)n + qq] = make_float4(0.f, 0.f, 0.f, 0.f);
+            if (kTop2) {
+                float4 ru = make_float4(INFINITY, INFINITY, INFINITY, __int_as_float(kRunnerNone));
+                if (b.pos2 >= 0) {
+                    const float4 t2 = g.pts[b.pos2];
+                    ru = make_float4(t2.x, t2.y, t2.z, __int_as_float(b.pos2));
+                }
+                cache[qq] = make_float4(pp.x, pp.y, pp.z, b.pos >= 0 ? fminf(b.third, cov2) : -1.f);
+                cache[3 * (size_t)n + qq] = ru;
+            } else {
+                cache[qq] = make_float4(pp.x, pp.y, pp.z, b.pos >= 0 ? fminf(b.second, cov2) : -1.f);
+                cache[3 * (size_t)n + qq] = make_float4(0.f, 0.f, 0.f, __int_as_float(kRunnerOff));
+            }
         }
         if (hist0 && b.pos >= 0) atomicAdd(&sh[__float_as_uint(b.d2) >> shift0], 1u);
     };
     constexpr int kP = 256 / G;
     constexpr int kKeys = 2 * kMaxLevels + 2;
     __shared__ float4 un_p[kP], un_b[kP];
+    __shared__ float2 un_c[kTop2 ? kP : 1];
     __shared__ uint32_t un_l[kP];
     __shared__ uint32_t key_cnt[kKeys + 1];
     const int grp = (int)(threadIdx.x / G);
@@ -97,11 +108,11 @@
     uint32_t rnk = 0;
     if (q < n) {
         const int hv = hint ? (int)hraw : 0;
-        if (nearest_halo<G, false, true>(g, p, sub, gbase, -1, hv >= 2 ? hv - 2 : -1, b, cov, l, &lvl, &cov2)) {
+        if (nearest_halo<G, kTop2, true>(g, p, sub, gbase, -1, hv >= 2 ? hv - 2 : -1, b, cov, l, &lvl, &cov2)) {
             if (sub == 0) emit(q, p, b, lvl, cov2);
 #if !O3D_MATCH_REGROUP
         } else if (true) {
-            b = nearest_levels<G, true, false>(g, p, sub, gbase, l, b, cov, seg_lds + grp * kSegWords<G>, 0.f, &lvl, &cov2);
+            b = nearest_levels<G, true, kTop2>(g, p, sub, gbase, l, b, cov, seg_lds + grp * kSegWords<G>, 0.f, &lvl, &cov2);
             if (sub == 0) emit(q, p, b, lvl, cov2);
 #endif
         } else {
@@ -128,6 +139,7 @@
         un_p[at] = make_float4(p.x, p.y, p.z, cov);
         un_b[at] = make_float4(b.d2, __uint_as_float(b.idx), __int_as_float(b.pos), b.second);
         un_l[at] = (uint32_t)l | ((uint32_t)grp << 8);
+        if (kTop2) un_c[at] = make_float2(__int_as_float(b.pos2), b.third);
     }
     __syncthreads();
     if (grp < (int)key_cnt[kKeys]) {
@@ -142,7 +154,12 @@
         b2.second = eb.w;
         b2.pos2 = -1;
         b2.third = INFINITY;
-        b2 = nearest_levels<G, true, false>(g, p2, sub, gbase, (int)(el & 255u), b2, ep.w, seg_lds + grp * kSegWords<G>, 0.f, &lvl, &cov2);
+        if (kTop2) {
+            const float2 ec = un_c[grp];
+            b2.pos2 = __float_as_int(ec.x);
+            b2.third = ec.y;
+        }
+        b2 = nearest_levels<G, true, kTop2>(g, p2, sub, gbase, (int)(el & 255u), b2, ep.w, seg_lds + grp * kSegWords<G>, 0.f, &lvl, &cov2);
         if (sub == 0) emit(q2, p2, b2, lvl, cov2);
     }
     if (hist0) {
diff --git a/open3d_slam_private_amd/csrc/kernels_tail.hpp b/open3d_slam_private_amd/csrc/kernels_tail.hpp
--- a/open3d_slam_private_amd/csrc/kernels_tail.hpp
+++ b/open3d_slam_private_amd/csrc/kernels_tail.hpp
@@ -31,6 +31,7 @@
 constexpr int kTailSearchedWord = 193;
 constexpr int kTailItersWord = 194;
 constexpr int kTailCauseWord = 195;
+constexpr int kTailSwappedWord = 196;
 constexpr int kTailStampWord = 200;
 constexpr int kTailGroups = kTailThreads / 8;
 constexpr int kTailBins = 1024;
@@ -58,6 +59,7 @@
     int tile;
     int max_iters;
     float slack;
+    int swap;
     unsigned long long seq;
     unsigned long long timeout_ticks;
 };
@@ -475,7 +477,7 @@
         return;
     }
     const unsigned cnt_lane = lane < 8 ? (unsigned)((nwg - lane + 7) >> 3) : 0u;
-    unsigned n_searched = 0;
+    unsigned n_searched = 0, n_swapped = 0;
     int exit_reason = 0;
     int k_local = 0;
     unsigned epoch = 0;
@@ -608,27 +610,11 @@
             bool pass = false;
             const float attr_ok = kGicp ? st_rows[4 * kTailSlots + sl].w : nn.w;
             if (valid[u] && c.w > 0.f && pprev >= 0 && attr_ok == 1.f) {
-                const float dx = p[u].x - tq.x, dy = p[u].y - tq.y, dz = p[u].z - tq.z;
-                float a = dx * dx;
-                float b2 = dy * dy;
-                float d2 = a + b2;
-                a = dz * dz;
-                d2 = d2 + a;
-                const float ex = p[u].x - c.x, ey = p[u].y - c.y, ez = p[u].z - c.z;
-                const float delta = __builtin_amdgcn_sqrtf(ex * ex + ey * ey + ez * ez);
-                const float lhs = (__builtin_amdgcn_sqrtf(d2) + delta) * 1.00001f + 1e-30f;
-                const float rhs = __builtin_amdgcn_sqrtf(c.w) * 0.99999f;
-                pass = d2 <= g.max_d2 && lhs < rhs;
-                if (ru.w == 1.f) {
-                    const float fx = p[u].x - ru.x, fy = p[u].y - ru.y, fz = p[u].z - ru.z;
-                    float a2 = fx * fx;
-                    float b3 = fy * fy;
-                    float r2 = a2 + b3;
-                    a2 = fz * fz;
-                    r2 = r2 + a2;
-                    pass = pass && d2 < r2;
-                }
-                if (pass) d2s[sl] = d2;
+                const Shortcut sc = shortcut_rule(p[u].x, p[u].y, p[u].z, c.x, c.y, c.z, c.w, tq.x, tq.y, tq.z, ru.x, ru.y, ru.z,
+                                                  __float_as_int(ru.w), g.max_d2, cfg.swap != 0);
+                pass = sc.outcome != kShortcutSearch;
+                if (pass) d2s[sl] = sc.d2;
+                if (sc.outcome == kShortcutSwap) fail[kTailSlots - 1 - (int)atomicAdd(&misc[1], 1u)] = (uint16_t)sl;
             }
             if (valid[u] && !pass) {
                 const unsigned at = atomicAdd(&misc[0], 1u);
@@ -690,8 +676,27 @@
             tq.w = __int_as_float(pos);
             st_rows[kTailSlots + slot] = tq;
             st_rows[2 * kTailSlots + slot] = nn;
-            st_rows[3 * kTailSlots + slot] = pos2 >= 0 ? make_float4(t2.x, t2.y, t2.z, 1.f)
-                                                       : make_float4(INFINITY, INFINITY, INFINITY, 1.f);
+            st_rows[3 * kTailSlots + slot] = pos2 >= 0 ? make_float4(t2.x, t2.y, t2.z, __int_as_float(pos2))
+                                                       : make_float4(INFINITY, INFINITY, INFINITY, __int_as_float(kRunnerNone));
+        }
+        const int ns = __builtin_amdgcn_readfirstlane((int)misc[1]);
+        n_swapped += (unsigned)ns;
+#pragma unroll 1
+        for (int si = tv; si < ns; si += kTailThreads) {
+            const int slot = (int)fail[kTailSlots - 1 - si];
+            const float4 nw = st_rows[3 * kTailSlots + slot], old = st_rows[kTailSlots + slot];
+            const size_t pc = (size_t)__float_as_int(nw.w);
+            float4 nn = kGicp ? tgt_nrm[2 * pc] : tgt_nrm[2 * pc + 1];
+            if (kGicp) {
+                float4 c1 = tgt_nrm[2 * pc + 1];
+                c1.w = 1.f;
+                st_rows[4 * kTailSlots + slot] = c1;
+            } else {
+                nn.w = 1.f;
+            }
+            st_rows[kTailSlots + slot] = nw;
+            st_rows[2 * kTailSlots + slot] = nn;
+            st_rows[3 * kTailSlots + slot] = old;
         }
         __syncthreads();
         TAIL_STAMP(1);
@@ -790,6 +795,7 @@
         }
         if (t == 0) {
             misc[0] = 0u;
+            misc[1] = 0u;
             misc[5] = 0u;
             misc[9] = 0u;
             misc[2] = __float_as_uint(INFINITY);
@@ -1076,7 +1082,14 @@
             }
         }
     }
-    if (t == 0 && n_searched) atomicAdd(&sync[kTailSearchedWord], n_searched);
+    if (t == 0 && n_searched) {
+        atomicAdd(&sync[kTailSearchedWord], n_searched);
+        atomicAdd(&it_g->tail_searched, (unsigned long long)n_searched);
+    }
+    if (t == 0 && n_swapped) {
+        atomicAdd(&sync[kTailSwappedWord], n_swapped);
+        atomicAdd(&it_g->tail_swapped, (unsigned long long)n_swapped);
+    }
 #if O3D_TAIL_STAMPS
     if (t == 0 && (blockIdx.x == 0 || blockIdx.x == gridDim.x - 1)) {
         unsigned long long* out = reinterpret_cast<unsigned long long*>(sync + kTailStampWord) + (blockIdx.x == 0 ? 0 : 12);
@@ -1118,7 +1131,7 @@
     if (lane < kSums) reinterpret_cast<HostMirror*>(mir_w)->sums[lane] = sit->sums[lane];
     __builtin_amdgcn_fence(__ATOMIC_ACQ_REL, "workgroup");
     __builtin_amdgcn_wave_barrier();
-    for (int w2 = lane; w2 < kStateWords; w2 += 64) reinterpret_cast<uint32_t*>(it_g)[w2] = s_state[w2];
+    for (int w2 = lane; w2 < kIterStateCopyWords; w2 += 64) reinterpret_cast<uint32_t*>(it_g)[w2] = s_state[w2];
     constexpr int kMirrorWords = (int)(offsetof(HostMirror, seq) / 4);
     uint32_t* hw = reinterpret_cast<uint32_t*>(host);
     for (int w2 = lane; w2 < kMirrorWords; w2 += 64) hw[w2] = mir_w[w2];
diff --git a/open3d_slam_private_amd/csrc/reg_state.hpp b/open3d_slam_private_amd/csrc/reg_state.hpp
--- a/open3d_slam_private_amd/csrc/reg_state.hpp
+++ b/open3d_slam_private_amd/csrc/reg_state.hpp
@@ -36,7 +36,9 @@
     float xicp_enough, xicp_insufficient, xicp_cos_min, xicp_cos_strong;
     float xicp_Trd[12];
     double xicp_comb[6], xicp_high[6];
+    unsigned long long tail_searched, tail_swapped;
 };
+constexpr int kIterStateCopyWords = (int)(offsetof(IterState, tail_searched) / 4);
 
 struct XicpState {
     float vr[9], vt[9];
@@ -107,6 +109,51 @@
     }
     return b;
 }
+constexpr int kRunnerNone = -1;
+constexpr int kRunnerOff = -2;
+enum ShortcutOutcome : int { kShortcutSearch = 0, kShortcutKeep = 1, kShortcutSwap = 2 };
+struct Shortcut {
+    int outcome;
+    float d2;
+};
+__host__ __device__ inline float shortcut_sqrt(float x) {
+#if defined(__HIP_DEVICE_COMPILE__)
+    return __builtin_amdgcn_sqrtf(x);
+#else
+    return sqrtf(x);
+#endif
+}
+__host__ __device__ inline float shortcut_d2(float px, float py, float pz, float qx, float qy, float qz) {
+    const float dx = px - qx, dy = py - qy, dz = pz - qz;
+    float a = dx * dx;
+    float b = dy * dy;
+    float d2 = a + b;
+    a = dz * dz;
+    d2 = d2 + a;
+    return d2;
+}
+__host__ __device__ inline Shortcut shortcut_rule(float px, float py, float pz, float ax, float ay, float az, float g2, float bx,
+                                                  float by, float bz, float rx, float ry, float rz, int rpos, float max_d2,
+                                                  bool allow_swap) {
+    float d2 = shortcut_d2(px, py, pz, bx, by, bz);
+    const float ex = px - ax, ey = py - ay, ez = pz - az;
+    const float delta = shortcut_sqrt(ex * ex + ey * ey + ez * ez);
+    const float lhs = (shortcut_sqrt(d2) + delta) * 1.00001f + 1e-30f;
+    const float rhs = shortcut_sqrt(g2) * 0.99999f;
+    bool keep = d2 <= max_d2 && lhs < rhs, swap = false;
+    if (rpos >= 0) {
+        const float r2 = shortcut_d2(px, py, pz, rx, ry, rz);
+        keep = keep && d2 < r2;
+        if (allow_swap) {
+            const float lhs2 = (shortcut_sqrt(r2) + delta) * 1.00001f + 1e-30f;
+            swap = r2 < d2 && r2 <= max_d2 && lhs2 < rhs;
+            if (swap) d2 = r2;
+        }
+    }
+    const Shortcut s = {swap ? kShortcutSwap : (keep ? kShortcutKeep : kShortcutSearch), d2};
+    return s;
+}
+
 constexpr int kQueues = 64;
 constexpr int kQueueStride = 16;
 
```
